# RustAudio/rodio

Measured on AMD Instinct MI355X. Metric: Msamples/s through resample+low_pass+mix pipeline, higher is better.
Workload: dtype f32; 1 GPU; 256 f32 stereo sources/GPU x 1048576 frames, 44.1->48 kHz linear resample + low_pass(200) + ordered Mixer sum, span_len=None; numpy default_rng(1234+s) U(-1,1)/256; in_frames=1048576, out_frames=1141308, channels=2, kernel=k_rlm_chunk

## Files before the change

### include/rodio_hip.h

```cpp
#ifndef RODIO_HIP_H
#define RODIO_HIP_H

#include <stddef.h>
#include <stdint.h>

#ifdef __cplusplus
extern "C" {
#endif

typedef int32_t rh_status;
enum {
    RH_OK = 0,
    RH_ERR_INVALID = 1,
    RH_ERR_HIP = 2,
    RH_ERR_UNSUPPORTED = 3,
    RH_ERR_NOMEM = 4,
    RH_ERR_TIMEOUT = 5,
    RH_ERR_NOT_INITIALIZED = 6,
    RH_ERR_CAPACITY = 7
};

typedef void *rh_stream;

int32_t rh_version(void);
// ... 172 lines not shown
    float knee_width_db;
    uint64_t attack_ns;
    uint64_t release_ns;
} rh_limit_params;
rh_status rh_limit(float *dst, const float *src, uint64_t frames, uint32_t channels,
                   uint32_t sample_rate, uint32_t n_streams, const rh_limit_params *params_host,
                   float *state, rh_stream stream);

typedef struct rh_agc_params {
    float target_level;
    uint64_t attack_ns;
    uint64_t release_ns;
    float absolute_max_gain;
    float floor;
} rh_agc_params;
size_t rh_agc_state_floats(void);
rh_status rh_agc_state_init(float *state, uint32_t n_streams, rh_stream stream);
rh_status rh_agc(float *dst, const float *src, uint64_t n_samples, uint32_t sample_rate,
                 uint32_t n_streams, const rh_agc_params *params_host, float *state,
                 rh_stream stream);

typedef struct rh_rlm_config {
    uint32_t from_rate, to_rate;
    uint32_t channels;
    uint64_t span_len;
    int32_t filter_kind;
    uint32_t filter_freq;
    float filter_q;
    uint32_t max_sources;
    uint64_t max_in_frames;
    uint32_t frames_per_lane;
    uint32_t ring_stages;
    uint32_t no_balance;
    uint32_t force_general;
    float custom_coeffs[5];
    uint32_t filter_first;
} rh_rlm_config;
typedef struct rh_rlm rh_rlm;
rh_status rh_rlm_create(rh_rlm **out, const rh_rlm_config *cfg);
rh_status rh_rlm_destroy(rh_rlm *p);
rh_status rh_rlm_set_sources(rh_rlm *p, const float *const *srcs_host,
                             const uint64_t *in_frames_host, uint32_t n_sources);
rh_status rh_rlm_set_gains(rh_rlm *p, const float *gains_host, uint32_t n);
rh_status rh_rlm_set_filters(rh_rlm *p, const int32_t *kinds_host, const uint32_t *freqs_host, const float *qs_host, uint32_t n);
rh_status rh_rlm_set_exclusive(rh_rlm *p, int32_t exclusive);
rh_status rh_rlm_set_mix_first(rh_rlm *p, int32_t enable);
rh_status rh_rlm_run(rh_rlm *p, float *dst, uint64_t out_capacity_frames, uint64_t *out_frames,
                     rh_stream stream);
rh_status rh_rlm_run_subset(rh_rlm *p, uint32_t first, uint32_t count, float *dst,
                            uint64_t out_capacity_frames, uint64_t *out_frames, rh_stream stream);
rh_status rh_rlm_stream_begin(rh_rlm *p);
rh_status rh_rlm_stream_block(rh_rlm *p, const float *const *srcs_host, uint32_t n_sources,
                              uint64_t avail_frames, int32_t flush, float *dst,
                              uint64_t out_capacity_frames, uint64_t *out_frames,
                              uint64_t *consumed_frames, rh_stream stream);
rh_status rh_rlm_stream_block_v(rh_rlm *p, const float *const *srcs_host, const uint64_t *avail_frames_host,
                                const uint8_t *ended_host, uint32_t n_sources, float *dst,
                                uint64_t out_capacity_frames, uint64_t *out_frames,
                                uint64_t *consumed_frames, rh_stream stream);
rh_status rh_rlm_stream_keep_history(rh_rlm *p, int32_t on);
rh_status rh_rlm_stream_overlap(rh_rlm *p, int32_t on);
rh_status rh_rlm_stream_one_launch_blocks(rh_rlm *p, uint32_t *blocks);
rh_status rh_rlm_stream_overlapped_blocks(rh_rlm *p, uint32_t *blocks);
rh_status rh_rlm_stream_stats(rh_rlm *p, uint32_t *summed_blocks, uint32_t *per_source_blocks, uint32_t *recoveries);
rh_status rh_rlm_run_batch(rh_rlm *p, float *dst, uint64_t dst_stride_frames, uint64_t *out_frames,
                           rh_stream stream);
rh_status rh_rlm_autotune(rh_rlm *p, float *dst, uint64_t out_capacity_frames, rh_stream stream,
                          uint32_t *frames_per_lane, uint32_t *ring_stages);
rh_status rh_rlm_last_status(rh_rlm *p);
rh_status rh_rlm_late_carries(rh_rlm *p, uint64_t *count);
rh_status rh_rlm_phase_cycles(rh_rlm *p, double out8[8]);
typedef struct rh_rlm_geometry_info {
    uint32_t threads;
    uint32_t frames_per_lane;
    uint32_t ring_stages;
    uint32_t stage_kib;
    uint32_t lds_bytes;
    uint32_t lookback_tiles;
    uint32_t resident_waves_per_cu;
    uint32_t n_tiles;
    uint32_t general_kernel;
    uint32_t ragged_pair;
    uint32_t mix_first;
} rh_rlm_geometry_info;
rh_status rh_rlm_geometry(rh_rlm *p, rh_rlm_geometry_info *info);

enum { RH_GEN_SINE = 0, RH_GEN_TRIANGLE = 1, RH_GEN_SQUARE = 2, RH_GEN_SAWTOOTH = 3 };
rh_status rh_signal_generator_init(float state_host[2], uint32_t sample_rate, float frequency);
rh_status rh_signal_generator_seek(float *phase_host, uint32_t sample_rate, float frequency, uint64_t pos_ns);
float rh_signal_phase_advance(float phase, float phase_step, uint64_t n);
rh_status rh_signal_generate(float *dst, uint64_t ld, uint64_t n, float *states_dev, const int32_t *functions_dev,
                             uint32_t n_gens, rh_stream stream);
rh_status rh_chirp_total_samples(uint32_t sample_rate, uint64_t duration_ns, uint64_t *total);
rh_status rh_chirp_total_duration(uint32_t sample_rate, uint64_t total, uint64_t *secs, uint32_t *nanos);
rh_status rh_chirp(float *dst, uint64_t first, uint64_t n, uint64_t total, uint32_t sample_rate, float start_frequency,
                   float end_frequency, uint64_t *out_n, rh_stream stream);

enum {
    RH_NOISE_WHITE_UNIFORM = 0,
    RH_NOISE_WHITE_TRIANGULAR = 1,
    RH_NOISE_WHITE_GAUSSIAN = 2,
    RH_NOISE_PINK = 3,
    RH_NOISE_BLUE = 4,
    RH_NOISE_VIOLET = 5,
    RH_NOISE_BROWNIAN = 6,
    RH_NOISE_RED = 7,
    RH_NOISE_VELVET = 8
};
rh_status rh_noise_init(uint32_t state_host[8], int32_t kind, uint32_t sample_rate, uint64_t seed, uint32_t density);
rh_status rh_noise_generate(float *dst, uint64_t ld, uint64_t n, uint32_t *states_dev, uint32_t n_streams, rh_stream stream);

typedef struct rh_comm rh_comm;
rh_status rh_comm_unique_id(uint8_t out128[128]);
rh_status rh_comm_init(rh_comm **out, int32_t rank, int32_t nranks, const uint8_t uid128[128]);
rh_status rh_comm_destroy(rh_comm *c);
rh_status rh_allreduce_sum_f32(rh_comm *c, float *buf, size_t n, rh_stream stream);
rh_status rh_reduce_sum_f32(rh_comm *c, float *buf, size_t n, int32_t root, rh_stream stream);

#ifdef __cplusplus
}
#endif
#endif
```

### rodio_amd/_lib.py

```python
from __future__ import annotations

import ctypes as C
import os

_HERE = os.path.dirname(os.path.abspath(__file__))
LIB_PATH = os.environ.get("RODIO_HIP_LIB") or os.path.join(_HERE, "librodio_hip.so")

RH_OK = 0
STATUS_NAMES = {
    0: "RH_OK", 1: "RH_ERR_INVALID", 2: "RH_ERR_HIP", 3: "RH_ERR_UNSUPPORTED", 4: "RH_ERR_NOMEM",
    5: "RH_ERR_TIMEOUT", 6: "RH_ERR_NOT_INITIALIZED", 7: "RH_ERR_CAPACITY",
}


class RhError(RuntimeError):
    def __init__(self, status: int, where: str, detail: str = ""):
        self.status = status
        super().__init__(f"{where}: {STATUS_NAMES.get(status, status)} {detail}".strip())


class LimitParams(C.Structure):
    _fields_ = [("threshold_db", C.c_float), ("knee_width_db", C.c_float),
                ("attack_ns", C.c_uint64), ("release_ns", C.c_uint64)]


class AgcParams(C.Structure):
    _fields_ = [("target_level", C.c_float), ("attack_ns", C.c_uint64), ("release_ns", C.c_uint64),
                ("absolute_max_gain", C.c_float), ("floor", C.c_float)]


class WavInfo(C.Structure):
    _fields_ = [("channels", C.c_uint32), ("sample_rate", C.c_uint32), ("bits_per_sample", C.c_uint32), ("is_float", C.c_int32),
                ("data_offset", C.c_uint64), ("data_bytes", C.c_uint64), ("samples", C.c_uint64)]


class UniformSeg(C.Structure):
    _fields_ = [("src", C.c_void_p), ("dst", C.c_void_p), ("src_frame0", C.c_uint64), ("src_frames", C.c_uint64), ("m0", C.c_uint64), ("m1", C.c_uint64),
                ("span_frames", C.c_uint64), ("from_rate", C.c_uint32), ("to_rate", C.c_uint32), ("from_ch", C.c_uint32), ("to_ch", C.c_uint32), ("gain", C.c_float), ("reserved", C.c_uint32)]


class WideSrc(C.Structure):
    _fields_ = [("data", C.c_void_p), ("channels", C.c_uint32), ("from_rate", C.c_uint32), ("phase", C.c_uint32), ("frames", C.c_uint64), ("last", C.c_uint32), ("gain", C.c_float)]


class RlmConfig(C.Structure):
    _fields_ = [("from_rate", C.c_uint32), ("to_rate", C.c_uint32), ("channels", C.c_uint32),
                ("span_len", C.c_uint64), ("filter_kind", C.c_int32), ("filter_freq", C.c_uint32),
                ("filter_q", C.c_float), ("max_sources", C.c_uint32), ("max_in_frames", C.c_uint64),
                ("frames_per_lane", C.c_uint32), ("ring_stages", C.c_uint32), ("no_balance", C.c_uint32), ("force_general", C.c_uint32), ("custom_coeffs", C.c_float * 5), ("filter_first", C.c_uint32)]


class RlmGeometry(C.Structure):
    _fields_ = [(n, C.c_uint32) for n in ("threads", "frames_per_lane", "ring_stages", "stage_kib", "lds_bytes",
                                           "lookback_tiles", "resident_waves_per_cu", "n_tiles", "general_kernel", "ragged_pair", "mix_first")]


vp, sz, u32, u64, i32, f32 = C.c_void_p, C.c_size_t, C.c_uint32, C.c_uint64, C.c_int32, C.c_float
f32p = C.POINTER(C.c_float)

SIGNATURES = {
    "rh_version": (i32, []),
    "rh_status_string": (C.c_char_p, [i32]),
    "rh_last_hip_error": (C.c_char_p, []),
    "rh_async_status": (i32, []),
    "rh_init": (i32, [i32]),
    "rh_device_name": (i32, [C.c_char_p, sz]),
    "rh_bind_thread": (i32, []),
    "rh_malloc": (i32, [C.POINTER(vp), sz]),
    "rh_free": (i32, [vp]),
    "rh_memset": (i32, [vp, i32, sz, vp]),
    "rh_memcpy_h2d": (i32, [vp, vp, sz, vp]),
    "rh_memcpy_h2d_rows": (i32, [vp, vp, sz, sz, sz, vp]),
    "rh_memcpy_d2h": (i32, [vp, vp, sz, vp]),
    "rh_memcpy_d2h_async": (i32, [vp, vp, C.c_size_t, vp]),
    "rh_memcpy_d2d": (i32, [vp, vp, C.c_size_t, vp]),
    "rh_host_alloc": (i32, [C.POINTER(vp), C.c_size_t]),
    "rh_host_free": (i32, [vp]),
    "rh_event_synchronize": (i32, [vp]),
    "rh_stream_wait_event": (i32, [vp, vp]),
    "rh_stream_create": (i32, [C.POINTER(vp)]),
    "rh_stream_destroy": (i32, [vp]),
    "rh_stream_synchronize": (i32, [vp]),
    "rh_stream_release_scratch": (i32, [vp]),
    "rh_event_create": (i32, [C.POINTER(vp)]),
    "rh_event_destroy": (i32, [vp]),
    "rh_event_record": (i32, [vp, vp]),
    "rh_event_elapsed_ms": (i32, [vp, vp, f32p]),
    "rh_convert_i8_to_f32": (i32, [vp, vp, sz, vp]),
    "rh_convert_u8_to_f32": (i32, [vp, vp, sz, vp]),
    "rh_convert_i16_to_f32": (i32, [vp, vp, sz, vp]),
    "rh_convert_u16_to_f32": (i32, [vp, vp, sz, vp]),
    "rh_convert_i24_to_f32": (i32, [vp, vp, sz, vp]),
    "rh_convert_i32_to_f32": (i32, [vp, vp, sz, vp]),
    "rh_convert_f32_to_i8": (i32, [vp, vp, sz, vp]),
    "rh_convert_f32_to_i16": (i32, [vp, vp, sz, vp]),
    "rh_convert_f32_to_u16": (i32, [vp, vp, sz, vp]),
    "rh_convert_f32_to_i32": (i32, [vp, vp, sz, vp]),
    "rh_convert_f32_to_u8": (i32, [vp, vp, sz, vp]),
    "rh_convert_f32_to_i24": (i32, [vp, vp, sz, vp]),
    "rh_convert_f32_to_u24": (i32, [vp, vp, sz, vp]),
    "rh_convert_f32_to_u32": (i32, [vp, vp, sz, vp]),
    "rh_convert_f32_to_i64": (i32, [vp, vp, sz, vp]),
    "rh_convert_f32_to_u64": (i32, [vp, vp, sz, vp]),
    "rh_convert_f32_to_f64": (i32, [vp, vp, sz, vp]),
    "rh_convert_u24_to_f32": (i32, [vp, vp, sz, vp]),
    "rh_convert_u32_to_f32": (i32, [vp, vp, sz, vp]),
    "rh_convert_i64_to_f32": (i32, [vp, vp, sz, vp]),
    "rh_convert_u64_to_f32": (i32, [vp, vp, sz, vp]),
    "rh_convert_f64_to_f32": (i32, [vp, vp, sz, vp]),
    "rh_channels_convert": (i32, [vp, vp, sz, u32, u32, vp]),
    "rh_amplify": (i32, [vp, vp, sz, f32, vp]),
    "rh_channel_volume": (i32, [vp, vp, sz, u32, f32p, u32, vp]),
    "rh_spatial_gains": (i32, [f32p, f32p, f32p, f32p]),
    "rh_periodic_update_samples": (u64, [u64, u32, u32]),
    "rh_amplify_steps": (i32, [vp, vp, sz, u64, u64, vp, u32, vp]),
    "rh_channel_volume_steps": (i32, [vp, vp, sz, u32, u32, u64, u64, vp, u32, u64, u64, vp, u32, vp]),
    "rh_delay_samples": (u64, [u64, u32, u32]),
    "rh_echo_mix": (i32, [vp, vp, sz, sz, f32, vp]),
    "rh_resample_out_frames": (i32, [u64, u32, u32, u32, u64, C.POINTER(u64)]),
    "rh_resample_linear": (i32, [vp, vp, u64, u32, u32, u32, u64, vp]),
    "rh_uniform_span_frames": (i32, [u64, u32, u32, i32, C.POINTER(u64)]),
    "rh_uniform_first_tap": (i32, [u64, u32, u32, C.POINTER(u64)]),
    "rh_uniform_cut_tail_samples": (i32, [u64, u32, u32, u32, u32, u32, C.POINTER(u64)]),
    "rh_uniform_segments": (i32, [C.POINTER(UniformSeg), u32, vp]),
    "rh_uniform_segments_dev": (i32, [vp, u32, u64, vp]),
    "rh_mix_sum": (i32, [vp, sz, C.POINTER(vp), C.POINTER(u64), C.POINTER(u64), u32, vp]),
    "rh_wide_mix_block": (i32, [vp, u32, u32, u64, C.POINTER(WideSrc), u32, vp]),
    "rh_biquad_coeffs": (i32, [i32, u32, f32, u32, f32p]),
    "rh_biquad": (i32, [vp, vp, u64, u32, u32, f32p, vp, i32, vp]),
    "rh_limit": (i32, [vp, vp, u64, u32, u32, u32, C.POINTER(LimitParams), vp, vp]),
    "rh_agc_state_floats": (sz, []),
    "rh_agc_state_init": (i32, [vp, u32, vp]),
    "rh_agc": (i32, [vp, vp, u64, u32, u32, C.POINTER(AgcParams), vp, vp]),
    "rh_resampler_create": (i32, [C.POINTER(vp), u32, u32, u32]),
    "rh_resampler_reset": (i32, [vp]),
    "rh_resampler_destroy": (i32, [vp]),
    "rh_resampler_pending_frames": (i32, [vp, u64, i32, C.POINTER(u64)]),
# ... 86 lines not shown
```

### rodio_amd/csrc/rh_common.h

```cpp
#pragma once
#include <mutex>
#include <hip/hip_runtime.h>

#include <cstdint>
#include <cstdio>

#include "../../include/rodio_hip.h"

namespace rh {

extern bool g_initialized;
extern int g_device;
extern int g_num_cus;
extern uint32_t *g_async_status;
void set_hip_error(hipError_t e, const char *what);

enum Knob {
    K_AGC_SEQ, K_AGC_VEC, K_BIQUAD_NO_FALLBACK, K_BIQUAD_SEQ, K_BIQUAD_R, K_BIQUAD_NW, K_BIQUAD_WGS, K_LIMIT_SEQ, K_LIMIT_R, K_LIMIT_NW, K_LIMIT_WGS, K_LIMIT_GRID,
    K_LIMIT_SKEW, K_LIMIT_NIO, K_LIMIT_INIT, K_SCAN_DMA_TOP, K_SCAN_SPIN_LIMIT, K_NO_HYBRID, K_NO_TICKET_SHARDS, K_PROF_DUMP, K_HOST_ALLOC, K_NO_MIX_FIRST, K_MIX_U, K_NO_CHUNK, K_CHUNK_HALF, K_AUTOTUNE_LOG, K_RAG_RESIDENT, K_RAG_TWO_KERNELS, K_AGC_SEGMENTS, K_RS_PIPE, K_DASP_I64_VIA_F64, K_MIX_GROUPS, K_CLASSES_SIDE_BY_SIDE, K_AGC_FUSED_R4, K_STREAM_UPLOAD_ALWAYS, K_STREAM_NO_REJOIN, K_NO_SBLK, K_SBLK_KV, K_SBLK_NO_OVERLAP, K_CLASSES_ONE_BY_ONE, K_CLASSES_ONE_WAVE, K_WIDE_GENERAL, K_PCM_NO_TILE, K_PCM_TILE_KB, K_LERP_IEEE_DIV, K_COUNTER_JUMP, K_STREAM_START, K_COUNT
};
const char *knob(Knob k);
void load_knobs();
struct CounterJump {
    bool on;
    uint32_t after, tickets_left, launches_left;
};
const CounterJump &counter_jump();
bool scan_jump_due();

#define RH_HIP_TRY(expr)                                   \
    do {                                                   \
        hipError_t _e = (expr);                            \
        if (_e != hipSuccess) {                            \
            ::rh::set_hip_error(_e, #expr);                \
            return RH_ERR_HIP;                             \
        }                                                  \
    } while (0)

#define RH_REQUIRE_INIT()                                  \
    do {                                                   \
        if (!::rh::g_initialized) return RH_ERR_NOT_INITIALIZED; \
    } while (0)

#define RH_CHECK_LAUNCH()                                  \
    do {                                                   \
        hipError_t _e = hipGetLastError();                 \
        if (_e != hipSuccess) {                            \
            ::rh::set_hip_error(_e, "kernel launch");      \
            return RH_ERR_HIP;                             \
        }                                                  \
    } while (0)

inline hipStream_t as_stream(rh_stream s) { return reinterpret_cast<hipStream_t>(s); }

inline hipError_t fill_now(void *p, int value, size_t bytes) {
    hipError_t e = hipMemset(p, value, bytes);
    return e != hipSuccess ? e : hipStreamSynchronize(nullptr);
}

hipError_t fill_async(void *p, int value, size_t bytes, hipStream_t s);
hipError_t counters_add(uint32_t *ctl, uint32_t d_ticket, uint32_t n_shards, uint32_t d_shards, hipStream_t s);

struct ScratchAux {
    uint64_t tag;
    uint32_t ticket_base;
    uint32_t parity;
};
hipError_t stream_scratch(hipStream_t s, size_t bytes, void **out, std::unique_lock<std::mutex> &hold, ScratchAux **aux = nullptr);
hipError_t copy_d2d(void *dst, const void *src, size_t bytes, hipStream_t hs);
bool lerp_div_fast_ok(uint32_t T);
inline float lerp_rcp(uint32_t T) { return lerp_div_fast_ok(T) ? 1.0f / (float)T : 0.0f; }
bool pcm_tile_try(float *dst, const uint8_t *data, uint64_t n_samples, uint64_t frames, uint32_t channels, uint32_t to_channels, int fmt, hipStream_t s);
void rlm_stream_retired(hipStream_t s);

inline unsigned grid_for(size_t work_items, unsigned block = 256, unsigned max_blocks = 256 * 8) {
    size_t b = (work_items + block - 1) / block;
    if (b < 1) b = 1;
    if (b > max_blocks) b = max_blocks;
    return static_cast<unsigned>(b);
}

inline unsigned grid_tiles(size_t vectors, unsigned block = 256) { return grid_for(vectors, block, 1u << 22); }

#ifdef __HIPCC__
typedef float nt_f4 __attribute__((ext_vector_type(4)));
typedef unsigned nt_u4 __attribute__((ext_vector_type(4)));
__device__ __forceinline__ float4 ld_nt(const float4 *p) {
    const nt_f4 v = __builtin_nontemporal_load(reinterpret_cast<const nt_f4 *>(p));
    return make_float4(v.x, v.y, v.z, v.w);
}
__device__ __forceinline__ uint4 ld_nt(const uint4 *p) {
    const nt_u4 v = __builtin_nontemporal_load(reinterpret_cast<const nt_u4 *>(p));
    return make_uint4(v.x, v.y, v.z, v.w);
}
__device__ __forceinline__ float ld_nt(const float *p) { return __builtin_nontemporal_load(p); }
__device__ __forceinline__ void st_nt(float4 *p, float4 v) {
    nt_f4 t;
    t.x = v.x; t.y = v.y; t.z = v.z; t.w = v.w;
    __builtin_nontemporal_store(t, reinterpret_cast<nt_f4 *>(p));
}
__device__ __forceinline__ void st_nt(float *p, float v) { __builtin_nontemporal_store(v, p); }

// ... 49 lines not shown
```

### rodio_amd/csrc/rh_pipeline.hip

```cpp
#include "rh_pipeline_dev.h"

namespace {


__device__ __forceinline__ uint32_t rag_find_pairs(const Params &p, const uint32_t m_tile0, const uint32_t m_stable, const int lane, lds_u8 *lds, const uint32_t list_off);
template <int R, int KV, int C>
__device__ __forceinline__ void rag_run_pairs(const Params &p, unsigned long long *const rows, const uint32_t tile, const uint32_t n_pairs, const int lane, lds_u8 *lds, const uint32_t lds0,
                                              const uint32_t list_off, const uint32_t i_base, const uint32_t nvec, const uint32_t (&goff)[KV], const int (&offA)[R + 2], const float (&wgt)[R + 2],
                                              const float (&lM)[4], const float (&b15)[4], const float (&b31)[4], const float (&kM)[4], typename Chan<C>::V (&acc)[R]);

template <int R, int KV, int NS, bool FILT, bool RAG = false, int C = 2, bool SUMF = false>
__global__ __launch_bounds__(64, (R <= 4 ? (KV <= 5 ? 5 : 4) : R <= 6 ? 3 : R <= 12 ? 2 : 1)) void k_rlm_fast(const Params p) {
    typedef Chan<C> CH;
    typedef typename CH::V V;
    constexpr uint32_t FB = CH::kFB, VF = CH::kVF;
    static_assert(R <= kMaxR, "frames per lane");
    static_assert(NS >= 2 && NS <= 4, "ring depth");
    static_assert(KV * (NS - 1) < 64, "vmcnt range");
    constexpr uint32_t kStage = KV * 1024;
    extern __shared__ __attribute__((aligned(16))) unsigned char smem[];
    lds_u8 *const lds = (lds_u8 *)smem;
    const uint32_t lds0 = (uint32_t)(uintptr_t)lds;

    const int lane = threadIdx.x;
// ... 1194 lines not shown
    for (int k = 0; k < KV; ++k) acc[k] = v4f{0.f, 0.f, 0.f, 0.f};
    if (v0 < nvec) {
#pragma unroll
        for (int d = 0; d < NS - 1; ++d)
            if ((uint32_t)d < n_sources) stage_source(d, d);
        uint32_t st = 0;
        float g_next = n_sources ? dgain[4] : 0.f;
        for (uint32_t s_ = 0; s_ < n_sources; ++s_) {
            const float g = g_next;
            g_next = s_ + 1 < n_sources ? dgain[8 * (uint64_t)(s_ + 1) + 4] : 0.f;
            if (s_ + NS - 1 < n_sources) {
                uint32_t into = st + NS - 1;
                into = into >= (uint32_t)NS ? into - NS : into;
                stage_source(s_ + NS - 1, into);
                wait_vm<KV *(NS - 1)>();
            } else {
                const uint32_t left = n_sources - 1 - s_;
                wait_groups<KV, NS>((int)left);
            }
            const lds_u8 *buf = lds + st * kStage;
            v4f v[KV];
#pragma unroll
            for (int k = 0; k < KV; ++k) v[k] = *(const lds_f4 *)(buf + k * 1024 + lane * 16);
            asm volatile("s_waitcnt lgkmcnt(0)" ::: "memory");
#pragma unroll
            for (int k = 0; k < KV; ++k) {
                acc[k].x = fma_(g, v[k].x, acc[k].x);
                acc[k].y = fma_(g, v[k].y, acc[k].y);
                acc[k].z = fma_(g, v[k].z, acc[k].z);
                acc[k].w = fma_(g, v[k].w, acc[k].w);
            }
            st = st + 1 == (uint32_t)NS ? 0 : st + 1;
        }
        wait_vm<0>();
#pragma unroll
        for (int k = 0; k < KV; ++k) {
            const uint64_t j = v0 + (uint64_t)k * 64 + lane;
            if (j < nvec) *reinterpret_cast<v4f *>(y + 4 * j) = acc[k];
        }
    }
    if (blockIdx.x == 0) {
        const uint64_t t = nvec * 4 + lane;
        if (t < n_floats) {
            float a = 0.f;
            for (uint32_t s_ = 0; s_ < n_sources; ++s_) a = fma_(dgain[8 * (uint64_t)s_ + 4], ((glb_cf32 *)(uintptr_t)(desc[4 * (uint64_t)s_] + src_off))[t], a);
            y[t] = a;
        }
        if (lane == 0) {
            ydesc->data = desc_row;
            ydesc->frames = frames;
            ydesc->out_frames = out_frames;
            ydesc->gain = 1.0f;
            ydesc->pad[0] = ydesc->pad[1] = ydesc->pad[2] = 0;
        }
    }
}

struct ChunkArgs {
    const uint32_t *m_lo;
    unsigned long long *halo;
    const float *lookT;
    const float *powM;
    const float *uni;
};
constexpr uint32_t kChunkMultiMax = 7;
struct ChunkMulti {
    struct Entry {
        Params p;
        ChunkArgs q;
    };
    uint32_t n;
    uint32_t first[kChunkMultiMax + 1];
    float *sum_out;
    Entry e[kChunkMultiMax];
};
static_assert(sizeof(ChunkMulti) <= 4096, "the kernarg segment");
#if defined(RH_CHUNK_DIAG) && RH_CHUNK_DIAG == 3
#define RH_CPH(i) { const unsigned long long cph_now = __builtin_readcyclecounter(); if (lane == 0) atomicAdd(p.ticket + 8 + (i), (uint32_t)(cph_now - cph_last)); cph_last = cph_now; }
#define RH_CPH_DECL unsigned long long cph_last = __builtin_readcyclecounter();
#else
#define RH_CPH(i)
#define RH_CPH_DECL
#endif
template <int R, int C, int KV>
__device__ __forceinline__ void rlm_chunk_tile(const Params &p, const ChunkArgs &q, const uint32_t block) {
    typedef Chan<C> CH;
    typedef typename CH::V V;
    constexpr int NS = 2, H = 4;
    constexpr uint32_t FB = CH::kFB;
    constexpr uint32_t kStage = KV * 1024, P = kStage / FB;
    constexpr uint32_t MB = NS * kStage + 64;
    __shared__ __attribute__((aligned(1024))) unsigned char smem[MB + kStage + 64];
    lds_u8 *const lds = (lds_u8 *)smem;
    const uint32_t lds0 = (uint32_t)(uintptr_t)lds;
    typedef __attribute__((address_space(4))) const uint64_t cu64;
    typedef __attribute__((address_space(4))) const float cf32;
    typedef __attribute__((address_space(4))) const uint32_t cu32;
    cu64 *const desc = (cu64 *)(uintptr_t)p.srcs;
    cf32 *const dgain = (cf32 *)(uintptr_t)p.srcs;
    const int lane = threadIdx.x;
    uint32_t tile = block;
    if (!p.direct) {
        const uint32_t x = block & 7u;
        const uint32_t k = __builtin_amdgcn_readfirstlane(lane == 0 ? atomicAdd(p.ticket + 32u * (1u + x), 1u) - p.shard_base : 0u);
        tile = x + 8u * k;
        if (tile >= p.n_tiles) return;
    }
#ifdef RH_CHUNK_RAGSIM
    const uint32_t Ns = p.eq_frames;
    const uint32_t S = 2u * tile < p.n_tiles ? p.n_sources : (uint32_t)(((uint64_t)p.n_sources * 2u * (p.n_tiles - tile)) / p.n_tiles);
#else
    const uint32_t Ns = p.eq_frames, S = p.n_sources;
#endif
    const uint32_t m_lo = ((cu32 *)(uintptr_t)q.m_lo)[tile], m_hi = ((cu32 *)(uintptr_t)q.m_lo)[tile + 1];
    const uint32_t m0 = m_lo + (uint32_t)lane * R;
    int nfl;
    uint32_t n_t_v;
    float pwv[4];
    {
        const uint32_t n_t = m_hi - m_lo;
        nfl = (int)n_t - lane * R < 0 ? 0 : ((int)n_t - lane * R > R ? R : (int)n_t - lane * R);
        const uint32_t nl0 = (n_t + R - 1) / R;
        const uint32_t v = nl0 ? n_t - (nl0 - 1) * R : 0;
        n_t_v = n_t;
        asm volatile("v_mov_b32 %0, %1" : "=v"(n_t_v) : "s"(n_t));
        const float *pw = q.powM + 4 * v;
#pragma unroll
        for (int k = 0; k < 4; ++k) {
            pwv[k] = pw[k];
            asm volatile("" : "+v"(pwv[k]));
        }
    }
    const bool first = (m0 == 0);

    const uint32_t nvec = Ns * C / 4;
    const uint32_t v0 = tile * (KV * 64);
    uint32_t goff[KV];
#pragma unroll
    for (int k = 0; k < KV; ++k) {
        uint32_t j = v0 + (uint32_t)k * 64 + lane;
        j = j < nvec ? j : nvec - 1;
        goff[k] = j * 16;
    }
    const bool lin = v0 + (uint32_t)(KV * 64) <= nvec;
    auto stage_source = [&](uint32_t s_, uint32_t stage) {
        const void *data = (const void *)(uintptr_t)desc[4 * (uint64_t)s_];
        if (lin) {
            glds16_run<KV>(data, goff[0], lds0 + stage * kStage);
        } else {
#pragma unroll
            for (int k = 0; k < KV; ++k) glds16(data, goff[k], lds0 + stage * kStage + k * 1024);
        }
    };
    if (S) stage_source(0, 0);
    if (S > 1) stage_source(1, 1);
    const Tables *__restrict__ tb = p.tabs;
    float lM[4], b15[4], b31[4], kM[4];
    constexpr int NHV = H * FB / 16;
    const uint32_t Jc = p.J < tile ? p.J : tile;
    int want_look = (uint32_t)lane < Jc ? 1 : 0;
    uint64_t a_halo_pub = (uint64_t)(uintptr_t)(q.halo + (uint64_t)tile * 8 + (uint32_t)(lane >= 64 - NHV ? lane - (64 - NHV) : 0) * 4);
    uint64_t a_halo_poll = (uint64_t)(uintptr_t)(q.halo + (uint64_t)(tile ? tile - 1 : 0) * 8 + (lane < H * C ? lane : 0));
    uint64_t a_gran_pub = (uint64_t)(uintptr_t)(p.gran + (uint64_t)tile * 4 + (lane < 2 * C ? lane : 0));
    uint64_t a_gran_poll = (uint64_t)(uintptr_t)(p.gran + (uint64_t)(tile ? tile - 1 - (want_look ? lane : 0) : 0) * 4);
    uint64_t a_out = (uint64_t)(uintptr_t)(p.out + ((uint64_t)m_lo + (uint32_t)lane) * C);
    uint32_t epoch_v = p.epoch;
    float U = q.uni[lane < 61 ? lane : 60];
    asm volatile("" : "+v"(want_look), "+v"(a_halo_pub), "+v"(a_halo_poll), "+v"(a_gran_pub), "+v"(a_gran_poll), "+v"(a_out), "+v"(epoch_v), "+v"(U));
    {
        const uint32_t Jc0 = Jc;
        const float *kp = q.lookT + ((uint64_t)tile * p.J + ((uint32_t)lane < Jc0 ? lane : 0)) * 4;
#pragma unroll
        for (int k = 0; k < 4; ++k) {
            lM[k] = tb->laneM[lane][k];
            b15[k] = tb->bc15M[lane][k];
            b31[k] = tb->bc31M[lane][k];
            kM[k] = kp[k];
        }
    }
    int offA[R + 2];
    float wgt[R + 2];
    {
        const int64_t fbase = (int64_t)tile * P;
        Cursor c = cursor_at(first ? 0 : m0 - 2, p);
#pragma unroll
        for (int rr = 0; rr < R + 2; ++rr) {
#if defined(RH_CHUNK_DIAG) && RH_CHUNK_DIAG == 2
            offA[rr] = (int)MB + rr * 8;
            wgt[rr] = 0.5f;
            continue;
#endif
            const bool dummy = first && rr < 2;
            uint64_t i;
            uint32_t num;
            cursor_resolve(c, p, i, num);
            if (i + 1 >= Ns) {
                i = Ns - 1;
                num = 0;
            }
            int64_t f = (int64_t)i - fbase;
            f = f < -H ? -H : (f > (int64_t)P - 1 ? (int64_t)P - 1 : f);
            offA[rr] = dummy ? (int)MB : (int)MB + (int)f * (int)FB;
            wgt[rr] = dummy ? 0.0f : (float)num / p.Tf;
            if (!dummy) cursor_next(c, p);
        }
    }
    v4f acc[KV];
#pragma unroll
    for (int k = 0; k < KV; ++k) acc[k] = v4f{0.f, 0.f, 0.f, 0.f};
    {
        uint32_t st = 0;
        float g_next = S ? dgain[4] : 0.f;
        for (uint32_t s_ = 0; s_ < S; ++s_) {
            const float g = g_next;
            g_next = s_ + 1 < S ? dgain[8 * (uint64_t)(s_ + 1) + 4] : 0.f;
            if (s_ + 1 < S) wait_vm<KV>();
            else wait_vm<0>();
            const lds_u8 *buf = lds + st * kStage;
            v4f v[KV];
#pragma unroll
            for (int k = 0; k < KV; ++k) v[k] = *(const lds_f4 *)(buf + k * 1024 + lane * 16);
            asm volatile("s_waitcnt lgkmcnt(0)" ::: "memory");
            if (s_ + 2 < S) stage_source(s_ + 2, st);
#pragma unroll
            for (int k = 0; k < KV; ++k) {
                acc[k].x = fma_(g, v[k].x, acc[k].x);
                acc[k].y = fma_(g, v[k].y, acc[k].y);
                acc[k].z = fma_(g, v[k].z, acc[k].z);
                acc[k].w = fma_(g, v[k].w, acc[k].w);
            }
            st ^= 1u;
        }
    }
    RH_CPH_DECL
#if defined(RH_CHUNK_DIAG) && RH_CHUNK_DIAG < 3
    {
        float t = 0.f;
#pragma unroll
        for (int k = 0; k < KV; ++k) t += acc[k].x + acc[k].y + acc[k].z + acc[k].w;
#pragma unroll
        for (int rr = 0; rr < R + 2; ++rr) t += wgt[rr] + (float)offA[rr];
        p.out[(uint64_t)tile * 64 + lane] = t + lM[0] + b15[0] + b31[0] + kM[0] + (float)nfl + (first ? 1.f : 0.f);
        return;
    }
#endif
    if (lane >= 64 - NHV) {
        unsigned long long *hp = (unsigned long long *)(uintptr_t)a_halo_pub;
        const float e[4] = {acc[KV - 1].x, acc[KV - 1].y, acc[KV - 1].z, acc[KV - 1].w};
#pragma unroll
        for (int w = 0; w < 4; ++w) __hip_atomic_store(hp + w, ((unsigned long long)epoch_v << 32) | __float_as_uint(e[w]), __ATOMIC_RELAXED, __HIP_MEMORY_SCOPE_AGENT);
    }
#pragma unroll
    for (int k = 0; k < KV; ++k) *(lds_f4 *)(lds + MB + (uint32_t)(k * 64 + lane) * 16) = acc[k];
    if (lane == 0) *(lds_f4 *)(lds + MB + kStage) = v4f{0.f, 0.f, 0.f, 0.f};
    bool dead = false;
    if (tile == 0) {
        if (lane < H * C) *(RH_LDS float *)(lds + MB - H * FB + lane * 4) = 0.0f;
    } else {
        const bool want = lane < H * C;
        const unsigned long long *hp = (const unsigned long long *)(uintptr_t)a_halo_poll;
        unsigned long long hv = 0;
        bool ok = false;
        uint32_t spins = 0;
        while (true) {
            if (want && !ok) {
                hv = __hip_atomic_load(hp, __ATOMIC_RELAXED, __HIP_MEMORY_SCOPE_AGENT);
                ok = (uint32_t)(hv >> 32) == epoch_v;
            }
            if (__all(ok || !want)) break;
            if (++spins > kSpinLimit) {
                if (lane == 0) atomicOr(p.status, 1u);
                dead = true;
                break;
            }
            __builtin_amdgcn_s_sleep(1);
        }
        if (want) *(RH_LDS float *)(lds + MB - H * FB + lane * 4) = dead ? __builtin_nanf("") : __uint_as_float((uint32_t)hv);
    }
    asm volatile("s_waitcnt lgkmcnt(0)" ::: "memory");
    __builtin_amdgcn_wave_barrier();
    RH_CPH(0)

    const float b0 = readlane_f(U, 0), c1 = readlane_f(U, 1), c2 = readlane_f(U, 2), na1 = -readlane_f(U, 3), na2 = -readlane_f(U, 4);
    V out[R];
    V E1 = CH::zero(), E2 = CH::zero();
    {
        V ta[R + 2], tb2[R + 2];
#pragma unroll
        for (int rr = 0; rr < R + 2; ++rr) {
            ta[rr] = CH::ld_lds(lds + offA[rr]);
            tb2[rr] = CH::ld_lds(lds + offA[rr] + FB);
        }
        auto tap = [&](int rr) -> V {
            V x;
#pragma unroll
            for (int ch = 0; ch < C; ++ch) CH::set(x, ch, fma_(CH::get(tb2[rr], ch) - CH::get(ta[rr], ch), wgt[rr], CH::get(ta[rr], ch)));
            return x;
        };
        V x2 = first ? CH::zero() : tap(0);
        V x1 = first ? CH::zero() : tap(1);
        V w1 = CH::zero(), w2 = CH::zero();
#pragma unroll
        for (int r = 0; r < R; ++r) {
            const V x = tap(r + 2);
            V w;
#pragma unroll
            for (int ch = 0; ch < C; ++ch) {
                const float wc = fma_(na1, CH::get(w1, ch), fma_(na2, CH::get(w2, ch), fma_(c2, CH::get(x2, ch), c1 * CH::get(x1, ch))));
                CH::set(w, ch, wc);
                CH::set(out[r], ch, fma_(b0, CH::get(x, ch), wc));
            }
            w2 = w1;
            w1 = w;
            x2 = x1;
            x1 = x;
            E1 = vsel(r + 1 == nfl, w1, E1);
            E2 = vsel(r + 1 == nfl, w2, E2);
        }
    }
    RH_CPH(1)
    float Pq[2 * C];
#pragma unroll
    for (int k = 0; k < 2 * C; ++k) Pq[k] = 0.f;
    {
        const float Tm[4] = {readlane_f(U, 5), readlane_f(U, 6), readlane_f(U, 7), readlane_f(U, 8)};
#pragma unroll
        for (int ch = 0; ch < C; ++ch) mat_acc(Tm, CH::get(E1, ch), CH::get(E2, ch), Pq[2 * ch], Pq[2 * ch + 1]);
    }
    float own[2 * C];
#pragma unroll
    for (int k = 0; k < 2 * C; ++k) own[k] = Pq[k];
#define RH_CSCAN(K, N)                                                                             \
    {                                                                                              \
        float sq[2 * C];                                                                           \
        _Pragma("unroll") for (int k = 0; k < 2 * C; ++k) sq[k] = dpp0<kDppRowShr + N, 0xf>(Pq[k]); \
        const float sM[4] = {readlane_f(U, 9 + 4 * K), readlane_f(U, 10 + 4 * K), readlane_f(U, 11 + 4 * K), readlane_f(U, 12 + 4 * K)}; \
        _Pragma("unroll") for (int ch = 0; ch < C; ++ch) mat_acc(sM, sq[2 * ch], sq[2 * ch + 1], Pq[2 * ch], Pq[2 * ch + 1]); \
    }
    RH_CSCAN(0, 1)
    RH_CSCAN(1, 2)
    RH_CSCAN(2, 4)
    RH_CSCAN(3, 8)
#undef RH_CSCAN
    {
        float sq[2 * C];
#pragma unroll
        for (int k = 0; k < 2 * C; ++k) sq[k] = dpp0<kDppBcast15, 0xa>(Pq[k]);
#pragma unroll
        for (int ch = 0; ch < C; ++ch) mat_acc(b15, sq[2 * ch], sq[2 * ch + 1], Pq[2 * ch], Pq[2 * ch + 1]);
    }
    {
        float sq[2 * C];
#pragma unroll
        for (int k = 0; k < 2 * C; ++k) sq[k] = dpp0<kDppBcast31, 0xc>(Pq[k]);
#pragma unroll
        for (int ch = 0; ch < C; ++ch) mat_acc(b31, sq[2 * ch], sq[2 * ch + 1], Pq[2 * ch], Pq[2 * ch + 1]);
    }
    {
        const uint32_t n_t = (uint32_t)__builtin_amdgcn_readfirstlane((int)n_t_v);
        const int nl = (int)((n_t + R - 1) / R);
        float A[2 * C];
#pragma unroll
        for (int k = 0; k < 2 * C; ++k) A[k] = 0.f;
        if (nl >= 1) {
#pragma unroll
            for (int k = 0; k < 2 * C; ++k) A[k] = __int_as_float(__builtin_amdgcn_readlane(__float_as_int(own[k]), nl - 1));
        }
        if (nl >= 2) {
            const float M[4] = {readfirstlane_f(pwv[0]), readfirstlane_f(pwv[1]), readfirstlane_f(pwv[2]), readfirstlane_f(pwv[3])};
            float xp[2 * C];
#pragma unroll
            for (int k = 0; k < 2 * C; ++k) xp[k] = __int_as_float(__builtin_amdgcn_readlane(__float_as_int(Pq[k]), nl - 2));
#pragma unroll
            for (int ch = 0; ch < C; ++ch) mat_acc(M, xp[2 * ch], xp[2 * ch + 1], A[2 * ch], A[2 * ch + 1]);
        }
        if (lane < 2 * C) {
            float ev = A[0];
#pragma unroll
            for (int k = 1; k < 2 * C; ++k) ev = lane == k ? A[k] : ev;
            __hip_atomic_store((unsigned long long *)(uintptr_t)a_gran_pub, ((unsigned long long)epoch_v << 32) | __float_as_uint(ev), __ATOMIC_RELAXED, __HIP_MEMORY_SCOPE_AGENT);
        }
    }
    float Q[2 * C];
#pragma unroll
    for (int k = 0; k < 2 * C; ++k) Q[k] = dpp0<kDppWaveShr1, 0xf>(Pq[k]);
    RH_CPH(2)
    float c[2 * C];
#pragma unroll
    for (int k = 0; k < 2 * C; ++k) c[k] = 0.f;
    if (tile > 0) {
        const bool want = want_look != 0;
        const unsigned long long *gp = (const unsigned long long *)(uintptr_t)a_gran_poll;
        unsigned long long gv[2 * C];
#pragma unroll
        for (int k = 0; k < 2 * C; ++k) gv[k] = 0;
        bool ok = false;
        uint32_t spins = 0;
        while (true) {
            if (want && !ok) {
                bool all = true;
#pragma unroll
                for (int k = 0; k < 2 * C; ++k) {
                    gv[k] = __hip_atomic_load(gp + k, __ATOMIC_RELAXED, __HIP_MEMORY_SCOPE_AGENT);
                    all = all && ((uint32_t)(gv[k] >> 32) == epoch_v);
                }
                ok = all;
            }
            if (__all(ok || !want)) break;
            if (++spins > kSpinLimit) {
                if (lane == 0) atomicOr(p.status, 1u);
                dead = true;
                break;
            }
            __builtin_amdgcn_s_sleep(4);
        }
        if (lane == 0 && spins) atomicAdd(p.status + 1, spins);
        if (want && ok && !dead) {
#pragma unroll
            for (int ch = 0; ch < C; ++ch) mat_acc(kM, __uint_as_float((uint32_t)gv[2 * ch]), __uint_as_float((uint32_t)gv[2 * ch + 1]), c[2 * ch], c[2 * ch + 1]);
        }
#pragma unroll
        for (int k = 0; k < 2 * C; ++k) {
            c[k] += dpp0<kDppRowShr + 1, 0xf>(c[k]);
            c[k] += dpp0<kDppRowShr + 2, 0xf>(c[k]);
            c[k] += dpp0<kDppRowShr + 4, 0xf>(c[k]);
            c[k] += dpp0<kDppRowShr + 8, 0xf>(c[k]);
            c[k] = readlane_f(c[k], 15) + readlane_f(c[k], 31);
        }
    }
    if (dead) {
#pragma unroll
        for (int k = 0; k < 2 * C; ++k) c[k] = __builtin_nanf("");
    }
    RH_CPH(3)
#pragma unroll
    for (int ch = 0; ch < C; ++ch) mat_acc(lM, c[2 * ch], c[2 * ch + 1], Q[2 * ch], Q[2 * ch + 1]);
    constexpr uint32_t kRow = (R + 1) * FB;
    {
        lds_u8 *row = lds + (uint32_t)lane * kRow;
#pragma unroll
        for (int r = 0; r < R; ++r) {
            V y;
#pragma unroll
            for (int ch = 0; ch < C; ++ch) CH::set(y, ch, fma_(readlane_f(U, 25 + 2 * r), Q[2 * ch], fma_(readlane_f(U, 26 + 2 * r), Q[2 * ch + 1], CH::get(out[r], ch))));
            if (C == 2) *(lds_f2 *)(row + r * FB) = v2f{CH::get(y, 0), CH::get(y, C - 1)};
            else *(RH_LDS float *)(row + r * FB) = CH::get(y, 0);
        }
    }
    asm volatile("s_waitcnt lgkmcnt(0)" ::: "memory");
    __builtin_amdgcn_wave_barrier();
    {
        const uint32_t n_t = (uint32_t)__builtin_amdgcn_readfirstlane((int)n_t_v);
        float *ot = (float *)(uintptr_t)a_out;
        for (uint32_t f0 = 0; f0 < n_t; f0 += 64) {
            const uint32_t f = f0 + (uint32_t)lane;
            if (f < n_t) {
                const lds_u8 *src2 = lds + (f / R) * kRow + (f % R) * FB;
                if (C == 2) {
                    const v2f a = *(const lds_f2 *)src2;
                    *reinterpret_cast<float2 *>(ot + (uint64_t)f0 * 2) = make_float2(a.x, a.y);
                } else {
                    ot[f0] = *(const RH_LDS float *)src2;
                }
            }
        }
    }
    RH_CPH(4)
}
template <int R, int C, int KV>
__global__ __launch_bounds__(64, 2) void k_rlm_chunk(const Params p, const ChunkArgs q) {
    rlm_chunk_tile<R, C, KV>(p, q, blockIdx.x);
}
template <int R, int C, int KV>
__global__ __launch_bounds__(64, 2) void k_rlm_chunk_multi(const ChunkMulti m) {
    uint32_t k = 0;
#pragma unroll
    for (uint32_t i = 1; i < kChunkMultiMax; ++i) k += (i < m.n && blockIdx.x >= m.first[i]) ? 1u : 0u;
    uint32_t b0 = 0;
#pragma unroll
    for (uint32_t i = 1; i < kChunkMultiMax; ++i) b0 = (i == k) ? m.first[i] : b0;
    k = __builtin_amdgcn_readfirstlane(k);
    typedef const __attribute__((address_space(4))) unsigned char *cbytes;
    cbytes e = (cbytes)__builtin_amdgcn_kernarg_segment_ptr() + offsetof(ChunkMulti, e) + (size_t)k * sizeof(ChunkMulti::Entry);
    Params p;
    ChunkArgs q;
    typedef const __attribute__((address_space(4))) uint32_t *cwords;
    static_assert(sizeof(Params) % 4 == 0 && sizeof(ChunkArgs) % 4 == 0 && offsetof(ChunkMulti::Entry, q) % 4 == 0, "copied word by word");
    {
        cwords wp = (cwords)(e + offsetof(ChunkMulti::Entry, p)), wq = (cwords)(e + offsetof(ChunkMulti::Entry, q));
        uint32_t *dp = reinterpret_cast<uint32_t *>(&p), *dq = reinterpret_cast<uint32_t *>(&q);
#pragma unroll
        for (uint32_t i = 0; i < sizeof(Params) / 4; ++i) dp[i] = wp[i];
#pragma unroll
        for (uint32_t i = 0; i < sizeof(ChunkArgs) / 4; ++i) dq[i] = wq[i];
    }
    rlm_chunk_tile<R, C, KV>(p, q, blockIdx.x - b0);
}

#if defined(RH_CLS_DIAG) && RH_CLS_DIAG == 9
__device__ unsigned long long g_cls_stamp[2048 * 8 * 8];
#define RH_CLS_STAMP(i) { if (lane == 0 && tile < 2048 && k < 8) g_cls_stamp[((uint64_t)tile * 8 + k) * 8 + (i)] = wall_clock64(); }
#else
#define RH_CLS_STAMP(i)
#endif
#define RH_PARG(T, e, f) (*(const __attribute__((address_space(4))) T *)((e) + offsetof(ChunkMulti::Entry, p) + offsetof(Params, f)))
#define RH_QARG(T, e, f) (*(const __attribute__((address_space(4))) T *)((e) + offsetof(ChunkMulti::Entry, q) + offsetof(ChunkArgs, f)))
template <int R, int C, int KV>
__global__ __launch_bounds__(128, 2) void k_rlm_chunk_classes(const ChunkMulti m) {
    typedef Chan<C> CH;
    typedef typename CH::V V;
    constexpr int NS = 2, H = 4;
    constexpr uint32_t FB = CH::kFB;
    constexpr uint32_t kStage = KV * 1024, P = kStage / FB;
    constexpr uint32_t kCtl = NS * kStage;
    constexpr uint32_t kImg = kStage + 128;
    constexpr uint32_t MB0 = kCtl + 64 + 64;
    __shared__ __attribute__((aligned(1024))) unsigned char smem[kCtl + 64 + 2 * kImg];
    lds_u8 *const lds = (lds_u8 *)smem;
    const uint32_t lds0 = (uint32_t)(uintptr_t)lds;
    typedef __attribute__((address_space(4))) const uint64_t cu64;
    typedef __attribute__((address_space(4))) const float cf32;
    typedef __attribute__((address_space(4))) const uint32_t cu32;
    typedef const __attribute__((address_space(4))) unsigned char *cbytes;
    const cbytes kseg = (cbytes)__builtin_amdgcn_kernarg_segment_ptr();
    const int wave = __builtin_amdgcn_readfirstlane((int)(threadIdx.x >> 6));
    const int lane = (int)(threadIdx.x & 63u);
    const uint32_t n_cls = m.n;
    const Params &p0 = m.e[0].p;
    const uint32_t tile = blockIdx.x;
    const uint32_t Ns = p0.eq_frames;
    auto entry = [&](uint32_t k) -> cbytes { return kseg + offsetof(ChunkMulti, e) + (size_t)k * sizeof(ChunkMulti::Entry); };
    auto ctl_read = [&](uint32_t which) -> uint32_t {
        uint32_t v;
        asm volatile("ds_read_b32 %0, %1\n\ts_waitcnt lgkmcnt(0)" : "=v"(v) : "v"(lds0 + kCtl + which * 4) : "memory");
        return (uint32_t)__builtin_amdgcn_readfirstlane((int)v);
    };
    auto ctl_write = [&](uint32_t which, uint32_t v) {
        asm volatile("s_waitcnt lgkmcnt(0)" ::: "memory");
        if (lane == 0) *(RH_LDS uint32_t *)(lds + kCtl + which * 4) = v;
        asm volatile("s_waitcnt lgkmcnt(0)" ::: "memory");
    };
    if (wave == 0) {
        if (lane < 2) *(RH_LDS uint32_t *)(lds + kCtl + lane * 4) = 0u;
    }
    asm volatile("s_waitcnt lgkmcnt(0)\n\ts_barrier" ::: "memory");
    if (wave == 0) {
        const uint32_t nvec = Ns * C / 4;
        const uint32_t v0 = tile * (KV * 64);
        uint32_t goff[KV];
#pragma unroll
        for (int k = 0; k < KV; ++k) {
            uint32_t j = v0 + (uint32_t)k * 64 + lane;
            j = j < nvec ? j : nvec - 1;
            goff[k] = j * 16;
        }
        const bool lin = v0 + (uint32_t)(KV * 64) <= nvec;
        auto stage_source = [&](cu64 *desc, uint32_t s_, uint32_t stage) {
            const void *data = (const void *)(uintptr_t)desc[4 * (uint64_t)s_];
            if (lin) {
                glds16_run<KV>(data, goff[0], lds0 + stage * kStage);
            } else {
#pragma unroll
                for (int k = 0; k < KV; ++k) glds16(data, goff[k], lds0 + stage * kStage + k * 1024);
            }
        };
        constexpr int NHV = H * FB / 16;
        __builtin_amdgcn_s_setprio(3);
        uint32_t kc = 0, sc = 0;
        cu64 *ndesc = (cu64 *)(uintptr_t)RH_PARG(uint64_t, entry(0), srcs);
        uint32_t nS = RH_PARG(uint32_t, entry(0), n_sources);
        uint32_t nstage = 0;
        auto request_next = [&]() {
            if (kc >= n_cls) return false;
            stage_source(ndesc, sc, nstage);
            nstage ^= 1u;
            if (++sc == nS) {
                sc = 0;
                if (++kc < n_cls) {
                    ndesc = (cu64 *)(uintptr_t)RH_PARG(uint64_t, entry(kc), srcs);
// ... 735 lines not shown

const void *chunk_kernel(int R, uint32_t channels, int KV) {
    if (channels == 2 && R == 9 && KV == 4) return reinterpret_cast<const void *>(&k_rlm_chunk<9, 2, 4>);
    if (channels == 2 && R == 18 && KV == 8) return reinterpret_cast<const void *>(&k_rlm_chunk<18, 2, 8>);
    if (channels == 2 && R == 18 && KV == 4) return reinterpret_cast<const void *>(&k_rlm_chunk<18, 2, 4>);
    if (channels == 1 && R == 18 && KV == 4) return reinterpret_cast<const void *>(&k_rlm_chunk<18, 1, 4>);
    if (channels == 1 && R == 18 && KV == 2) return reinterpret_cast<const void *>(&k_rlm_chunk<18, 1, 2>);
    return nullptr;
}

static const void *chunk_multi_kernel(int R, uint32_t channels, int KV) {
    if (channels == 2 && R == 9 && KV == 4) return reinterpret_cast<const void *>(&k_rlm_chunk_multi<9, 2, 4>);
    if (channels == 2 && R == 18 && KV == 8) return reinterpret_cast<const void *>(&k_rlm_chunk_multi<18, 2, 8>);
    if (channels == 2 && R == 18 && KV == 4) return reinterpret_cast<const void *>(&k_rlm_chunk_multi<18, 2, 4>);
    if (channels == 1 && R == 18 && KV == 4) return reinterpret_cast<const void *>(&k_rlm_chunk_multi<18, 1, 4>);
    if (channels == 1 && R == 18 && KV == 2) return reinterpret_cast<const void *>(&k_rlm_chunk_multi<18, 1, 2>);
    return nullptr;
}

static const void *chunk_classes_kernel(int R, uint32_t channels, int KV) {
    if (channels == 2 && R == 18 && KV == 8) return reinterpret_cast<const void *>(&k_rlm_chunk_classes<18, 2, 8>);
    if (channels == 2 && R == 18 && KV == 4) return reinterpret_cast<const void *>(&k_rlm_chunk_classes<18, 2, 4>);
    if (channels == 1 && R == 18 && KV == 4) return reinterpret_cast<const void *>(&k_rlm_chunk_classes<18, 1, 4>);
    if (channels == 1 && R == 18 && KV == 2) return reinterpret_cast<const void *>(&k_rlm_chunk_classes<18, 1, 2>);
    return nullptr;
}

rh_status chunk_launch_classes(rh_rlm *const *classes, float *const *rows, uint64_t row_capacity_frames, uint32_t n, float *dst_sum, rh_stream stream, bool *taken, bool *summed) {
    *taken = false;
    *summed = false;
    if (n < 2 || n > kChunkMultiMax || rh::knob(rh::K_CLASSES_ONE_BY_ONE)) return RH_OK;
    const void *fn = nullptr;
    for (uint32_t k = 0; k < n; ++k) {
        const rh_rlm *h = classes[k];
        if (!h || !h->cls.empty() || !h->plan || h->out_frames == 0 || row_capacity_frames < h->out_frames) return RH_OK;
        if (!h->chunk.ok || !mix_first_applies(h, *h->plan, h->n_sources, false, false)) return RH_OK;
        const void *f = chunk_multi_kernel(h->chunk.R, h->cfg.channels, h->chunk.KV);
        if (!f || (fn && f != fn)) return RH_OK;
        fn = f;
    }
    ChunkMulti m;
    memset(&m, 0, sizeof m);
    for (uint32_t k = 0; k < n; ++k) {
        rh_rlm *h = classes[k];
        h->collect = &m;
        const rh_status st = rlm_launch(h, 0, h->n_sources, rows[k], row_capacity_frames, nullptr, stream, 0, 0, StreamArgs{});
        h->collect = nullptr;
        if (st != RH_OK) return st;
        if (m.n != k + 1) return RH_ERR_UNSUPPORTED;
    }
    void *args[] = {&m};
    hipStream_t s = rh::as_stream(stream);
    const void *fn2 = rh::knob(rh::K_CLASSES_ONE_WAVE) ? nullptr : chunk_classes_kernel(classes[0]->chunk.R, classes[0]->cfg.channels, classes[0]->chunk.KV);
    bool same = fn2 != nullptr;
    for (uint32_t k = 0; k < n && same; ++k) {
        const rh_rlm *h = classes[k], *h0 = classes[0];
        same = h->exclusive && h->eq_frames == h0->eq_frames && h->out_frames == h0->out_frames && h->F == h0->F && h->T == h0->T && h->chunk_in == h0->chunk_in &&
               h->chunk_out == h0->chunk_out && h->chunk.n_tiles == h0->chunk.n_tiles && h->chunk.R == h0->chunk.R && h->chunk.KV == h0->chunk.KV && h->n_sources >= 1;
    }
    if (same) {
        int per_cu = 0;
        same = hipOccupancyMaxActiveBlocksPerMultiprocessor(&per_cu, fn2, 128, 0) == hipSuccess && per_cu >= 1 &&
               (uint64_t)classes[0]->chunk.n_tiles <= (uint64_t)per_cu * (uint64_t)rh::g_num_cus;
    }
    hipError_t e;
    if (same) {
        m.sum_out = dst_sum;
        e = hipLaunchKernel(fn2, dim3(classes[0]->chunk.n_tiles), dim3(128), args, 0, s);
        *summed = e == hipSuccess;
    } else {
        e = hipLaunchKernel(fn, dim3(m.first[m.n]), dim3(64), args, 0, s);
        if (e == hipSuccess)
            for (uint32_t k = 0; k < n; ++k) classes[k]->shard_base += (m.first[k + 1] - m.first[k]) / 8u;
    }
    if (e != hipSuccess) {
        rh::set_hip_error(e, "k_rlm_chunk_multi / k_rlm_chunk_classes launch");
        return RH_ERR_HIP;
    }
    for (uint32_t k = 0; k < n; ++k) mark_launch(classes[k], s);
    *taken = true;
    return RH_OK;
}

#if defined(RH_CLS_DIAG) && RH_CLS_DIAG == 9
extern "C" int rh_debug_cls_stamps(unsigned long long *dst, size_t n) {
    return (int)hipMemcpyFromSymbol(dst, HIP_SYMBOL(g_cls_stamp), n * sizeof(unsigned long long), 0, hipMemcpyDeviceToHost);
}
#endif
void launch_state(hipStream_t s, unsigned long long *gran, const Tables *tabs, uint32_t n_sources, uint32_t cols, uint32_t last_col, uint32_t J, uint32_t epoch, uint32_t next_epoch) {
    hipLaunchKernelGGL(k_rlm_state, dim3((n_sources + 63) / 64), dim3(64), 0, s, gran, tabs, n_sources, cols, last_col, J, epoch, next_epoch);
}

void launch_state_sum(hipStream_t s, const unsigned long long *gran, const SrcDesc *srcs, uint32_t n_sources, uint32_t cols, uint32_t tag, float *w_out) {
    hipLaunchKernelGGL(k_rlm_state_sum, dim3(1), dim3(256), 0, s, gran, srcs, n_sources, cols, tag, w_out);
}

bool mix_first_applies(const rh_rlm *p, const Plan &pl, uint32_t count, bool per_source_states, bool batch) {
    return &pl == &p->fast && p->filt && p->mix_first_on && !per_source_states && !batch && count >= 2 && !rh::knob(rh::K_NO_MIX_FIRST);
}

rh_status rlm_launch(rh_rlm *p, uint32_t first, uint32_t count, float *dst, uint64_t out_capacity_frames, uint64_t *out_frames, rh_stream stream, uint32_t batch_streams, uint64_t out_stride,
                            const StreamArgs &sa) {
    RH_REQUIRE_INIT();
    if (!p) return RH_ERR_INVALID;
    if (!p->cls.empty()) return RH_ERR_UNSUPPORTED;
    if (first > p->n_sources || count > p->n_sources - first) return RH_ERR_INVALID;
    if (out_frames) *out_frames = p->out_frames;
    if (p->out_frames == 0) return RH_OK;
    if (!dst || (reinterpret_cast<uintptr_t>(dst) & 15u)) return RH_ERR_INVALID;
    if (out_capacity_frames < p->out_frames) return RH_ERR_CAPACITY;
    hipStream_t s = rh::as_stream(stream);
    {
        const rh_status w = pre_launch(p, s);
        if (w != RH_OK) return w;
    }
    const Plan &pl = *p->plan;
    {
        const rh_status w = next_epoch(p, s);
        if (w != RH_OK) return w;
    }
    Params k;
    k.srcs = p->d_srcs + first;
    k.tabs = pl.d_tabs;
    k.out = dst;
    k.gran = p->d_gran;
    k.ticket = p->d_ctl;
    k.status = p->d_ctl + 1;
    k.out_frames = p->out_frames;
    k.chunk_in = sa.mode ? p->st_chunk_in : p->chunk_in;
    k.chunk_out = sa.mode ? p->st_chunk_out : p->chunk_out;
    k.n_sources = count;
    k.n_tiles = p->n_tiles;
    k.F = p->F;
    k.T = p->T;
    k.qF = p->F / p->T;
    k.rF = p->F % p->T;
    k.Tf = (float)p->T;
    k.rcpT = rh::lerp_rcp(p->T);
    k.epoch = p->epoch;
    k.J = pl.J;
    k.ticket_base = p->ticket_base;
    k.direct = 0;
    k.rag_merge = k.rag_pairs_from = k.rag_pairs_to = 0;
    k.prof = p->d_prof;
    k.eq_frames = p->eq_frames;
    k.batch_streams = batch_streams;
    k.shards = (batch_streams >= 16 && batch_streams % 8 == 0 && !rh::knob(rh::K_NO_TICKET_SHARDS)) ? 8u : 1u;
    k.shard_base = p->shard_base;
    k.out_stride = out_stride;
    k.st_mode = sa.mode;
    k.st_active = sa.active;
    k.st_m0 = sa.m0;
    k.st_g0 = sa.g0;
    k.st_mfirst = sa.mode ? p->st_mfirst : 0;
    k.st_win = sa.win;
    k.st_wout = sa.wout;
    k.gran_cols = sa.gran_cols ? sa.gran_cols : p->n_tiles;
    k.col0 = sa.gran_cols ? 1u : 0u;
    k.u = pl.uni;
    void *args[] = {&k};
    const uint64_t grid = (uint64_t)p->n_tiles * (batch_streams ? batch_streams : 1);
    if (grid > 0x7fffffffull) return RH_ERR_UNSUPPORTED;
    if (&pl == &p->pair && !sa.mode && !batch_streams) {
        Params k1 = k;
        k1.gran = p->d_gran + (uint64_t)count * p->n_tiles * 4;
        k1.eq_frames = p->rag_frames;
        void *args1[] = {&k1};
#ifdef RH_RAG_NO_SUMF
        const bool merge = false;
#else
        const bool merge = !rh::knob(rh::K_RAG_TWO_KERNELS) || !pl.v->plain;
#endif
        k1.rag_merge = merge ? 1u : 0u;
        k1.rag_pairs_from = p->rag_pairs_from;
        k1.rag_pairs_to = p->rag_pairs_to;
        uint32_t lds1 = pl.lds_bytes + 128u;
        if (const char *w = rh::knob(rh::K_RAG_RESIDENT)) {
            const int want = atoi(w);
            if (want >= 2 && want < 8) lds1 = std::max(lds1, (kLdsGranules / (uint32_t)want) * kLdsGranule);
        }
        const uint32_t grid8 = ((uint32_t)grid + 7u) & ~7u;
        k1.shards = 8;
        k1.shard_base = p->shard_base;
        hipError_t e1 = hipLaunchKernel(reinterpret_cast<const void *>(pl.v->filt), dim3(grid8), dim3(64), args1, lds1, s);
        if (e1 == hipSuccess) p->shard_base += grid8 / 8u;
        if (e1 == hipSuccess && !merge) {
            k.ticket_base = p->ticket_base;
            e1 = hipLaunchKernel(reinterpret_cast<const void *>(pl.v->plain), dim3((uint32_t)grid), dim3(64), args, 2u * (uint32_t)pl.v->KV * 1024u + 128u , s);
            p->ticket_base += (uint32_t)grid;
        }
        if (e1 != hipSuccess) {
            rh::set_hip_error(e1, "ragged batch launch");
            return RH_ERR_HIP;
        }
        return mark_launch(p, s);
    }
    if (p->chunk.ok && !sa.mode && mix_first_applies(p, pl, count, false, batch_streams != 0) && count == p->n_sources && first == 0) {
        const ChunkPlan &c = p->chunk;
        k.tabs = c.d_tabs;
        k.gran = c.d_gran;
        k.n_tiles = c.n_tiles;
        k.J = c.J;
        k.u = c.uni;
        ChunkArgs ca;
        ca.m_lo = c.d_mlo;
        ca.halo = c.d_halo;
        ca.lookT = c.d_look;
        ca.powM = c.d_pow;
        ca.uni = c.d_uni;
        k.direct = (c.direct && p->exclusive) ? 1u : 0u;
        if (p->collect) {
            ChunkMulti &m = *static_cast<ChunkMulti *>(p->collect);
            if (m.n >= kChunkMultiMax) return RH_ERR_UNSUPPORTED;
            k.direct = 0;
            const uint32_t g8 = (c.n_tiles + 7u) & ~7u;
            m.e[m.n].p = k;
            m.e[m.n].q = ca;
            m.first[m.n + 1] = m.first[m.n] + g8;
            m.n += 1;
            return RH_OK;
        }
        const uint32_t cgrid = k.direct ? c.n_tiles : (c.n_tiles + 7u) & ~7u;
        void *cargs[] = {&k, &ca};
        const hipError_t ce = hipLaunchKernel(c.fn, dim3(cgrid), dim3(64), cargs, 0, s);
        if (ce != hipSuccess) {
            rh::set_hip_error(ce, "k_rlm_chunk launch");
            return RH_ERR_HIP;
        }
        if (!k.direct) p->shard_base += cgrid / 8u;
        return mark_launch(p, s);
    }
    const bool pre = p->pre_filter;
    if (pre && (&pl != &p->fast || sa.mode || batch_streams)) return RH_ERR_UNSUPPORTED;
    if (pre || mix_first_applies(p, pl, count, sa.gran_cols != 0, batch_streams != 0)) {
        const uint64_t n_floats = (uint64_t)p->eq_frames * p->cfg.channels;
        const size_t row = (size_t)(((sa.mode ? (uint64_t)p->cfg.max_in_frames * p->cfg.channels : n_floats) + 3) & ~3ull);
        constexpr uint32_t kMixGroups = 16;
        const uint64_t nvec = n_floats / 4;
        int U = 4;
        while (U > 1 && (nvec + 256ull * U - 1) / (256ull * U) < 2ull * (uint64_t)rh::g_num_cus) U /= 2;
        if (const char *u = rh::knob(rh::K_MIX_U)) U = atoi(u);
        const uint32_t per = 256u * (uint32_t)(U == 1 ? 1 : U == 2 ? 2 : 4);
        const uint32_t wgs = (uint32_t)std::max<uint64_t>(1, (nvec + per - 1) / per);
        const uint64_t ring_waves = (nvec + 511) / 512;
        int ring = ring_waves >= 2ull * rh::g_num_cus ? 2 : 0;
        if (const char *u = rh::knob(rh::K_MIX_U)) ring = atoi(u) >= 10 ? atoi(u) - 10 : 0;
        uint32_t groups = 1;
        const uint64_t per_cu = rh::knob(rh::K_MIX_GROUPS) ? (uint64_t)std::max(1, atoi(rh::knob(rh::K_MIX_GROUPS))) : 2ull;
        if (!pre && !ring && !rh::knob(rh::K_MIX_U))
            while (groups < kMixGroups && (uint64_t)wgs * groups < per_cu * (uint64_t)rh::g_num_cus && count / (groups * 2) >= 8) groups *= 2;
        const size_t rows_needed = pre ? 2 : (sa.mode ? kMixGroups : groups);
        const size_t need = row * rows_needed + 64 + kMixGroups * 8;
        if (need > p->mix_floats) {
            const rh_status w = wait_idle(p);
            if (w != RH_OK) return w;
            if (p->d_mix) RH_HIP_TRY(hipFree(p->d_mix));
            p->d_mix = nullptr;
            RH_HIP_TRY(hipMalloc(reinterpret_cast<void **>(&p->d_mix), need * sizeof(float)));
            p->mix_floats = need;
        }
        SrcDesc *const ydesc = reinterpret_cast<SrcDesc *>(p->d_mix + (p->mix_floats - 32 - kMixGroups * 8));
        float *const frow = pre ? p->d_mix + row : p->d_mix;
        const uint32_t nf = p->eq_frames, mf = (uint32_t)p->out_frames;
        if (ring >= 3) hipLaunchKernelGGL(k_mix_ring<3>, dim3((uint32_t)ring_waves), dim3(64), 0, s, k.srcs, count, p->d_mix, n_floats, ydesc, nf, mf, frow, sa.src_off);
        else if (ring == 2) hipLaunchKernelGGL(k_mix_ring<2>, dim3((uint32_t)ring_waves), dim3(64), 0, s, k.srcs, count, p->d_mix, n_floats, ydesc, nf, mf, frow, sa.src_off);
        else if (U == 1) hipLaunchKernelGGL(k_mix_rows<1>, dim3(wgs, groups), dim3(256), 0, s, k.srcs, count, p->d_mix, n_floats, ydesc, nf, mf, frow, (uint64_t)row, sa.src_off);
        else if (U == 2) hipLaunchKernelGGL(k_mix_rows<2>, dim3(wgs, groups), dim3(256), 0, s, k.srcs, count, p->d_mix, n_floats, ydesc, nf, mf, frow, (uint64_t)row, sa.src_off);
        else hipLaunchKernelGGL(k_mix_rows<4>, dim3(wgs, groups), dim3(256), 0, s, k.srcs, count, p->d_mix, n_floats, ydesc, nf, mf, frow, (uint64_t)row, sa.src_off);
        RH_CHECK_LAUNCH();
        if (pre) {
            const rh_status fs = rh_biquad(frow, p->d_mix, p->eq_frames, p->cfg.channels, 1, p->pre_coeffs, nullptr, 1, stream);
            if (fs != RH_OK) return fs;
        }
        k.srcs = ydesc;
        k.n_sources = groups;
        k.direct = (p->exclusive && (uint64_t)p->n_tiles <= (uint64_t)rh::g_num_cus * (uint64_t)std::max(pl.resident_per_cu, 0)) ? 1u : 0u;
    }
    hipError_t e = hipLaunchKernel(pl.kernel, dim3((uint32_t)grid), dim3(64), args, batch_streams ? std::max((uint32_t)pl.v->KV * 1024u, 64u * ((uint32_t)pl.v->R * 8u + 8u))  : p->launch_lds, s);
    if (e != hipSuccess) {
        rh::set_hip_error(e, "k_rlm launch");
        return RH_ERR_HIP;
    }
    if (k.direct) {}
    else if (k.shards > 1) p->shard_base += (uint32_t)(grid / k.shards);
    else p->ticket_base += (uint32_t)grid;
    return mark_launch(p, s);
}

}
```

### rodio_amd/csrc/rh_pipeline_internal.h

```cpp
#pragma once
#include <algorithm>
#include <cmath>
#include <cstddef>
#include <cstdio>
#include <cstdlib>
#include <cstring>
#include <mutex>
#include <numeric>
#include <type_traits>
#include <unordered_map>
#include <vector>

#include "rh_common.h"

namespace rh {
struct ResampleGeom {
    uint32_t F, T;
    uint64_t in_frames, chunk_in, chunk_out, n_chunks, last_in, out_frames;
    int fits32;
};
rh_status make_resample_geom(uint64_t in_frames, uint32_t from_rate, uint32_t to_rate, uint32_t channels, uint64_t span_len, ResampleGeom *g);
}

namespace rhp {

#ifndef RH_CARRY_DEFER
#define RH_CARRY_DEFER 2
#endif
constexpr int kMaxR = 20;
constexpr int kGroupLag = RH_CARRY_DEFER;
constexpr int kMaxLook = 32;
constexpr uint32_t kSpinLimit = 1u << 22;

struct SrcDesc {
    const float *data;
    uint32_t frames;
    uint32_t out_frames;
    float gain;
    uint32_t pad[3];
};
static_assert(sizeof(SrcDesc) == 32, "descriptor stride");

struct Uniforms {
    float b0, c1, c2, a1, a2;
    float Tm[4];
    float scanM[4][4];
    float g[kMaxR][2];
};
struct Tables {
    float bc15M[64][4];
    float bc31M[64][4];
    float laneM[64][4];
    float lookM[64][4];
};

struct Params {
    const SrcDesc *srcs;
    const Tables *tabs;
    float *out;
    unsigned long long *gran;
    uint32_t *ticket;
    uint32_t *status;
    uint64_t out_frames;
    uint64_t chunk_in, chunk_out;
    uint32_t n_sources, n_tiles;
    uint32_t F, T, qF, rF;
    float Tf, rcpT;
    uint32_t epoch, J;
    uint32_t ticket_base;
    uint32_t direct;
    unsigned long long *prof;
    uint32_t eq_frames;
    uint32_t batch_streams;
    uint32_t shards;
    uint32_t shard_base;
    uint64_t out_stride;
    uint32_t st_mode, st_active;
    uint64_t st_m0, st_g0;
    uint64_t st_mfirst;
    uint32_t gran_cols, col0;
    const float *st_win;
    float *st_wout;
    uint32_t rag_merge, rag_pairs_from, rag_pairs_to;
    Uniforms u;
};

struct M2 {
    double a, b, c, d;
};
inline M2 mul(const M2 &x, const M2 &y) { return {x.a * y.a + x.b * y.c, x.a * y.b + x.b * y.d, x.c * y.a + x.d * y.c, x.c * y.b + x.d * y.d}; }
inline M2 mpow(M2 base, uint64_t e) {
    M2 r{1, 0, 0, 1};
    while (e) {
        if (e & 1) r = mul(r, base);
        base = mul(base, base);
        e >>= 1;
    }
    return r;
}
inline void put(float *dst, const M2 &m) {
    dst[0] = (float)m.a;
    dst[1] = (float)m.b;
    dst[2] = (float)m.c;
    dst[3] = (float)m.d;
}
inline double norm(const M2 &m) { return std::fabs(m.a) + std::fabs(m.b) + std::fabs(m.c) + std::fabs(m.d); }

inline void scan_basis(double a1, double a2, M2 &T, M2 &Tinv) {
    const double disc = a1 * a1 - 4.0 * a2;
    const double re = -0.5 * a1;
    double mu, nu;
    if (disc < 0.0 && std::sqrt(-disc) * 0.5 > 1e-3) {
        mu = re;
        nu = std::sqrt(-disc) * 0.5;
    } else {
        const double sq = disc > 0.0 ? std::sqrt(disc) * 0.5 : 0.0;
        const double l1 = re + sq, l2 = re - sq;
        mu = std::fabs(l1) < std::fabs(l2) ? l1 : l2;
        nu = 1.0;
    }
    T = {1.0, -mu, 0.0, nu};
    Tinv = {1.0, mu / nu, 0.0, 1.0 / nu};
}

using KernelFn = void (*)(const Params);
struct Variant {
    int R, KV, NS;
    KernelFn filt, plain;
};
struct VariantTab {
    const Variant *v;
    size_t n;
};
template <size_t N>
constexpr VariantTab tab_of(const Variant (&t)[N]) { return VariantTab{t, N}; }
inline const Variant *find_variant(VariantTab tab, int R, int kv_needed, int NS) {
    const Variant *best = nullptr;
    for (size_t i = 0; i < tab.n; ++i) {
        const Variant &v = tab.v[i];
        if (v.R == R && v.NS == NS && v.KV >= kv_needed && (!best || v.KV < best->KV)) best = &v;
    }
    return best;
}
constexpr uint32_t kLdsGranule = 1280, kLdsGranules = 128;
inline int blocks_per_cu(const void *fn, size_t lds) {
    if (hipFuncSetAttribute(fn, hipFuncAttributeMaxDynamicSharedMemorySize, 160 * 1024 - 512) != hipSuccess) return 0;
    int n = 0;
    if (hipOccupancyMaxActiveBlocksPerMultiprocessor(&n, fn, 64, lds) != hipSuccess) return 0;
    const int by_lds = lds ? (int)(kLdsGranules / ((lds + kLdsGranule - 1) / kLdsGranule)) : n;
    return n < by_lds ? n : by_lds;
}
inline int kv_needed(uint64_t L, uint32_t F, uint32_t T, uint32_t channels) {
    const uint64_t fb = 4ull * channels, vf = 16 / fb;
    const uint64_t span = ((L + 1) * F) / T + 5 + (128 / fb - 2);
    const uint64_t nvec = span / vf + 2;
    return (int)((nvec + 63) / 64);
}

struct ChunkPlan {
    int R = 18, KV = 8;
    const void *fn = nullptr;
    int tabs_R = 0;
    bool ok = false;
    Uniforms uni;
    Tables *d_tabs = nullptr;
    float *d_pow = nullptr;
    float *d_uni = nullptr;
    uint32_t *d_mlo = nullptr;
    float *d_look = nullptr;
    unsigned long long *d_halo = nullptr;
    unsigned long long *d_gran = nullptr;
    size_t cap_tiles = 0, cap_look = 0;
    uint32_t n_tiles = 0, J = 0, frames = 0;
    int resident_per_cu = 0;
    bool direct = true;
};
struct Plan {
    const Variant *v = nullptr;
    const void *kernel = nullptr;
    bool general = false;
    uint32_t J = 0, lds_bytes = 0;
    int resident_per_cu = 0;
    Uniforms uni;
    Tables *d_tabs = nullptr;
};

struct StreamArgs {
    uint32_t mode = 0, active = 0;
    uint64_t m0 = 0, g0 = 0;
    const float *win = nullptr;
    float *wout = nullptr;
    uint32_t gran_cols = 0;
    uint64_t src_off = 0;
};
}
using namespace rhp;

struct rh_rlm {
    rh_rlm_config cfg;
    uint32_t F, T;
    uint64_t chunk_in, chunk_out;
    bool filt;
    float coeffs[5];
    Plan fast, wave;
    Plan pair;
    Plan *plan = nullptr;
    uint32_t launch_lds = 0;
    uint32_t rag_frames = 0;
    uint32_t rag_pairs_from = 0, rag_pairs_to = 0;
    uint32_t eq_frames = 0;
    bool equal = true;
    std::vector<Plan> tried;
    SrcDesc *d_srcs = nullptr;
    uint64_t srcs_version = 0;
    std::vector<const float *> st_tab_ptrs;
    uint64_t st_tab_version = ~0ull;
    unsigned long long *d_gran = nullptr;
    size_t gran_words = 0;
    uint32_t *d_ctl = nullptr;
    float *d_mix = nullptr;
    size_t mix_floats = 0;
    ChunkPlan chunk;
    bool cls_one_launch = false;
    void *collect = nullptr;
    void *sblk = nullptr;
    bool pre_filter = false;
    float pre_coeffs[5] = {1.f, 0.f, 0.f, 0.f, 0.f};
    unsigned long long *d_prof = nullptr;
    uint32_t n_sources = 0, n_tiles = 0;
    uint64_t out_frames = 0;
    uint32_t epoch = 0;
    uint32_t n_epochs = 0;
    uint32_t ticket_base = 0;
    uint32_t shard_base = 0;
    bool st_on = false, st_done = false;
    uint64_t st_g0 = 0, st_m = 0;
    uint64_t st_mfirst = 0;
    uint64_t st_chunk_in = 0, st_chunk_out = 0;
    uint32_t st_nsrc = 0;
    float *d_w[2] = {nullptr, nullptr};
    int st_cur = 0;
    std::vector<SrcDesc> h_desc;
    static constexpr int kDescRing = 4;
    SrcDesc *h_ring[kDescRing] = {nullptr, nullptr, nullptr, nullptr};
    hipEvent_t h_ring_ev[kDescRing] = {nullptr, nullptr, nullptr, nullptr};
    int h_ring_next = 0;
    std::vector<float> gains;
    std::vector<uint64_t> st_total;
    uint32_t st_cols = 0;
    bool st_history = false;
    bool st_together = false;
    bool st_dirty = false;
    bool st_decided = false;
    std::vector<const float *> st_prev_ptrs;
// ... 67 lines not shown
```

### rodio_amd/csrc/rh_pipeline_plan.hip

```cpp
#include "rh_pipeline_internal.h"

namespace {

std::mutex g_handles_mu;
std::vector<rh_rlm *> g_handles;
}

namespace rhp {

rh_status wait_idle(rh_rlm *p) {
    if (p->launched) {
        hipError_t e = hipSuccess;
        if (!p->idle_ev) e = hipEventCreateWithFlags(&p->idle_ev, hipEventDisableTiming);
        if (e == hipSuccess) e = hipEventRecord(p->idle_ev, p->last_stream);
        if (e == hipSuccess) e = hipEventSynchronize(p->idle_ev);
        if (e != hipSuccess) {
            (void)hipGetLastError();
            e = hipDeviceSynchronize();
        }
        p->launched = false;
        p->last_stream = nullptr;
        if (e != hipSuccess) {
            rh::set_hip_error(e, "wait_idle");
            return RH_ERR_HIP;
        }
    }
    return RH_OK;
}
rh_status pre_launch(rh_rlm *p, hipStream_t s) {
    if (p->launched && p->last_stream != s) return wait_idle(p);
    return RH_OK;
}
rh_status mark_launch(rh_rlm *p, hipStream_t s) {
    p->launched = true;
    p->last_stream = s;
    return RH_OK;
}

}
namespace {
__global__ void k_retag(unsigned long long *w, size_t n, uint32_t lo, uint32_t hi, uint32_t sub, uint32_t zero_below) {
    for (size_t i = (size_t)blockIdx.x * blockDim.x + threadIdx.x; i < n; i += (size_t)gridDim.x * blockDim.x) {
        const unsigned long long v = w[i];
        const uint32_t t = (uint32_t)(v >> 32);
        if (t == 0 || t > hi || (t < lo && !zero_below)) continue;
        const uint32_t u = t >= lo ? t - sub : 0u;
        w[i] = u ? ((unsigned long long)u << 32) | (v & 0xffffffffull) : 0ull;
    }
}
}
namespace rhp {
hipError_t launch_retag(unsigned long long *w, size_t n, const Retag &r, hipStream_t s) {
    if (!w || !n) return hipSuccess;
    hipLaunchKernelGGL(k_retag, dim3(rh::grid_for(n)), dim3(256), 0, s, w, n, r.lo, r.hi, r.sub, r.zero_below ? 1u : 0u);
    return hipGetLastError();
}
static rh_status retag_tables(rh_rlm *p, hipStream_t s, const Retag &r) {
    RH_HIP_TRY(launch_retag(p->d_gran, p->gran_words, r, s));
    RH_HIP_TRY(launch_retag(p->chunk.d_halo, p->chunk.cap_tiles * 8, r, s));
    RH_HIP_TRY(launch_retag(p->chunk.d_gran, p->chunk.cap_tiles * 4, r, s));
    sblk_retag(p, s, r);
    RH_CHECK_LAUNCH();
    return RH_OK;
}
rh_status next_epoch(rh_rlm *p, hipStream_t s, bool *launched) {
    if (launched) *launched = false;
    const rh::CounterJump &j = rh::counter_jump();
    if (j.on && ++p->n_epochs == j.after) {
        const uint32_t to = 0u - j.tickets_left;
        const uint32_t dt = to - p->ticket_base, ds = to - p->shard_base;
        RH_HIP_TRY(rh::counters_add(p->d_ctl, dt, 8u, ds, s));
        p->ticket_base += dt;
        p->shard_base += ds;
        const uint32_t target = kEpochLimit - (j.launches_left < kEpochLimit - 1 ? j.launches_left : kEpochLimit - 1);
        if (target > p->epoch) {
            const rh_status st = retag_tables(p, s, Retag{p->epoch + 1u, p->epoch + 1u, p->epoch - target, false});
            if (st != RH_OK) return st;
            p->epoch = target;
        }
        if (launched) *launched = true;
    }
    if (p->epoch >= kEpochLimit) {
        const rh_status st = retag_tables(p, s, Retag{kEpochShift + 1u, 0xffffffffu, kEpochShift, true});
        if (st != RH_OK) return st;
        p->epoch -= kEpochShift;
        if (launched) *launched = true;
    }
    p->epoch += 1;
    return RH_OK;
}

uint32_t look_tiles(const M2 &B, uint64_t L) {
    const M2 BL = mpow(B, L);
    M2 cur = BL;
    for (uint32_t j = 1; j <= (uint32_t)kMaxLook; ++j) {
        if (norm(cur) < 0x1p-40) return j;
        cur = mul(cur, BL);
    }
    return 0;
}
size_t lds_bytes_of(const Variant &v, bool general, uint32_t J) {
    size_t n = (size_t)v.NS * v.KV * 1024;
    if (general) n += 128 + 32 + kMaxLook * 16 + (size_t)((J + 3) / 4) * 1024;
    return n;
}

rh_status make_plan(rh_rlm *p, Plan &pl, VariantTab tab, bool general, const rh::ResampleGeom &g, uint32_t want_R, uint32_t want_NS) {
    const M2 A{-(double)p->coeffs[3], -(double)p->coeffs[4], 1.0, 0.0};
    M2 Tm, Ti;
    scan_basis((double)p->coeffs[3], (double)p->coeffs[4], Tm, Ti);
    const M2 B = mul(mul(Tm, A), Ti);
    const uint64_t M = g.out_frames ? g.out_frames : 1;
    const int cus = rh::g_num_cus;
    const double per_frame = 19.0, per_source = general ? 170.0 : 50.0;
    double best = 1e300;
    const Variant *bestV = nullptr;
    uint32_t bestJ = 0;
    for (int R = 1; R <= kMaxR; ++R) {
        if (want_R && (int)want_R != R) continue;
        const uint64_t L = 64ull * R;
        const uint32_t Jr = p->filt ? look_tiles(B, L) : 1;
        if (Jr == 0) continue;
        const uint64_t tiles = (M + L - 1) / L;
        const uint64_t per_cu = (tiles + cus - 1) / cus;
        for (int NS = 2; NS <= 4; ++NS) {
            if (want_NS && (int)want_NS != NS) continue;
            const Variant *v = find_variant(tab, R, kv_needed(L, g.F, g.T, p->cfg.channels), NS);
            if (!v) continue;
            const void *fn = reinterpret_cast<const void *>(p->filt ? v->filt : v->plain);
            const int resident = blocks_per_cu(fn, lds_bytes_of(*v, general, Jr));
            if (resident < 1) continue;
            const double passes = std::ceil((double)per_cu / resident);
            const uint64_t on_cu = std::min<uint64_t>(per_cu, resident);
            const double w = std::ceil(on_cu / 4.0);
            const double issue = 2.6 + 1.7 / std::pow(w, 1.5);
            double cost = passes * w * (per_frame * R + per_source) * issue;
            cost *= 1.0 + 0.01 * NS;
            if (general && R < 8) cost *= 1.3;
            if (cost < best) {
                best = cost;
                bestV = v;
                bestJ = Jr;
            }
// ... 107 lines not shown
        }
        if (fits) {
            R = in.R, KV = in.KV, fn = in.fn;
            break;
        }
    }
    if (!fn) return RH_OK;
    if (c.fn != fn) {
        int n = 0;
        if (hipOccupancyMaxActiveBlocksPerMultiprocessor(&n, fn, 64, 0) != hipSuccess) return RH_OK;
        c.resident_per_cu = n < 1 ? -1 : n;
        c.fn = fn;
        c.R = R;
        c.KV = KV;
    }
    if (c.resident_per_cu < 1) return RH_OK;
    c.direct = tiles <= (uint64_t)rh::g_num_cus * (uint64_t)c.resident_per_cu;
    const M2 A{-(double)p->coeffs[3], -(double)p->coeffs[4], 1.0, 0.0};
    M2 Tm, Ti;
    scan_basis((double)p->coeffs[3], (double)p->coeffs[4], Tm, Ti);
    const M2 B = mul(mul(Tm, A), Ti);
    const uint32_t J = look_tiles(B, n_min);
    if (J == 0 || J > 32) return RH_OK;
    if ((uint64_t)tiles * J * 16 > (64ull << 20)) return RH_OK;
    {
        const rh_status w = wait_idle(p);
        if (w != RH_OK) return w;
    }
    if (c.tabs_R != R) {
        if (c.d_tabs) RH_HIP_TRY(hipFree(c.d_tabs));
        if (c.d_pow) RH_HIP_TRY(hipFree(c.d_pow));
        if (c.d_uni) RH_HIP_TRY(hipFree(c.d_uni));
        c.d_tabs = nullptr, c.d_pow = nullptr, c.d_uni = nullptr, c.tabs_R = 0;
        Tables *h = new Tables();
        std::memset(h, 0, sizeof(Tables));
        Uniforms &U = c.uni;
        std::memset(&U, 0, sizeof(U));
        U.b0 = p->coeffs[0];
        U.c1 = (float)((double)p->coeffs[1] - (double)p->coeffs[0] * (double)p->coeffs[3]);
        U.c2 = (float)((double)p->coeffs[2] - (double)p->coeffs[0] * (double)p->coeffs[4]);
        U.a1 = p->coeffs[3];
        U.a2 = p->coeffs[4];
        put(U.Tm, Tm);
        for (int k = 0; k < 4; ++k) put(U.scanM[k], mpow(B, (uint64_t)R << k));
        for (int r = 0; r < R; ++r) {
            const M2 m = mul(mpow(A, r + 1), Ti);
            U.g[r][0] = (float)m.a;
            U.g[r][1] = (float)m.b;
        }
        for (int l = 0; l < 64; ++l) {
            put(h->laneM[l], mpow(B, (uint64_t)R * l));
            put(h->bc15M[l], mpow(B, (uint64_t)R * ((l & 15) + 1)));
            put(h->bc31M[l], mpow(B, (uint64_t)R * ((l & 31) + 1)));
        }
        float pw[kMaxR + 1][4];
        std::memset(pw, 0, sizeof(pw));
        for (int v = 0; v <= R; ++v) put(pw[v], mpow(B, (uint64_t)v));
        hipError_t e = hipMalloc(reinterpret_cast<void **>(&c.d_tabs), sizeof(Tables));
        if (e == hipSuccess) e = hipMemcpy(c.d_tabs, h, sizeof(Tables), hipMemcpyHostToDevice);
        if (e == hipSuccess) e = hipMalloc(reinterpret_cast<void **>(&c.d_pow), sizeof(pw));
        if (e == hipSuccess) e = hipMemcpy(c.d_pow, pw, sizeof(pw), hipMemcpyHostToDevice);
        static_assert(offsetof(Uniforms, Tm) == 20 && offsetof(Uniforms, scanM) == 36 && offsetof(Uniforms, g) == 100, "the kernel reads the Uniforms by float index");
        if (e == hipSuccess) e = hipMalloc(reinterpret_cast<void **>(&c.d_uni), sizeof(Uniforms));
        if (e == hipSuccess) e = hipMemcpy(c.d_uni, &U, sizeof(Uniforms), hipMemcpyHostToDevice);
        delete h;
        if (e != hipSuccess) {
            rh::set_hip_error(e, "k_rlm_chunk tables");
            return e == hipErrorOutOfMemory ? RH_ERR_NOMEM : RH_ERR_HIP;
        }
        c.tabs_R = R;
    }
    if ((size_t)tiles > c.cap_tiles) {
        if (c.d_mlo) RH_HIP_TRY(hipFree(c.d_mlo));
        if (c.d_halo) RH_HIP_TRY(hipFree(c.d_halo));
        if (c.d_gran) RH_HIP_TRY(hipFree(c.d_gran));
        c.d_mlo = nullptr, c.d_halo = nullptr, c.d_gran = nullptr, c.cap_tiles = 0;
        RH_HIP_TRY(hipMalloc(reinterpret_cast<void **>(&c.d_mlo), ((size_t)tiles + 1) * 4));
        RH_HIP_TRY(hipMalloc(reinterpret_cast<void **>(&c.d_halo), (size_t)tiles * 64));
        RH_HIP_TRY(hipMalloc(reinterpret_cast<void **>(&c.d_gran), (size_t)tiles * 32));
        RH_HIP_TRY(rh::fill_now(c.d_halo, 0, (size_t)tiles * 64));
        RH_HIP_TRY(rh::fill_now(c.d_gran, 0, (size_t)tiles * 32));
        c.cap_tiles = (size_t)tiles;
    }
    const size_t look_floats = (size_t)tiles * J * 4;
    if (look_floats > c.cap_look) {
        if (c.d_look) RH_HIP_TRY(hipFree(c.d_look));
        c.d_look = nullptr, c.cap_look = 0;
        RH_HIP_TRY(hipMalloc(reinterpret_cast<void **>(&c.d_look), look_floats * 4));
        c.cap_look = look_floats;
    }
    std::vector<float> look(look_floats, 0.0f);
    {
        std::unordered_map<uint64_t, M2> memo;
        for (uint64_t t = 1; t < tiles; ++t)
            for (uint32_t j = 0; j < J && j < t; ++j) {
                const uint64_t d = (uint64_t)mlo[(size_t)t] - mlo[(size_t)(t - j)];
                auto it = memo.find(d);
                if (it == memo.end()) it = memo.emplace(d, mpow(B, d)).first;
                put(&look[((size_t)t * J + j) * 4], it->second);
            }
    }
    RH_HIP_TRY(hipMemcpy(c.d_mlo, mlo.data(), mlo.size() * 4, hipMemcpyHostToDevice));
    RH_HIP_TRY(hipMemcpy(c.d_look, look.data(), look_floats * 4, hipMemcpyHostToDevice));
    c.n_tiles = (uint32_t)tiles;
    c.J = J;
    c.frames = (uint32_t)Ns;
    c.ok = true;
    return RH_OK;
}

bool pair_ok(rh_rlm *p, const Plan &pl) {
    if (!pl.v || !p->filt || p->equal || p->cfg.force_general || p->h_desc.size() != p->n_sources || rh::knob(rh::K_NO_HYBRID)) return false;
    const uint64_t M = p->out_frames, L = 64ull * pl.v->R, J = pl.J;
    const uint64_t tiles = (M + L - 1) / L;
    if (!tiles) return false;
    uint32_t frames_of_longest = 0, most = 0, ends_from = 0xffffffffu, ends_to = 0;
    std::vector<uint32_t> pairs((size_t)tiles, 0u);
    for (const SrcDesc &d : p->h_desc) {
        if (d.out_frames == M) {
            if (frames_of_longest && frames_of_longest != d.frames) return false;
            frames_of_longest = d.frames;
        } else if (d.out_frames > 0) {
            ends_from = std::min(ends_from, d.out_frames);
            ends_to = std::max(ends_to, d.out_frames);
            const uint64_t t_end = (d.out_frames - 1) / L;
            const uint64_t t_lo = (uint64_t)d.out_frames / L > J ? (uint64_t)d.out_frames / L - J : 0;
            for (uint64_t t = t_lo; t <= t_end && t < tiles; ++t) most = std::max(most, ++pairs[(size_t)t]);
        }
    }
    if (!frames_of_longest || most > 24) return false;
    p->rag_frames = frames_of_longest;
    p->rag_pairs_from = ends_from;
    p->rag_pairs_to = ends_to;
    return true;
}

rh_status activate_plan(rh_rlm *p, Plan *pl) {
    const uint64_t M = p->out_frames;
    const uint64_t L = 64ull * pl->v->R;
    const uint64_t tiles = (M + L - 1) / L;
    if (tiles > 0x7fffffffull) return RH_ERR_UNSUPPORTED;
    const size_t words = (size_t)(p->n_sources + 1) * (tiles + 1) * 4;
    if (p->filt && words > p->gran_words) {
        {
            const rh_status w = wait_idle(p);
            if (w != RH_OK) return w;
        }
        if (p->d_gran) RH_HIP_TRY(hipFree(p->d_gran));
        p->d_gran = nullptr;
        RH_HIP_TRY(hipMalloc(reinterpret_cast<void **>(&p->d_gran), words * 8));
        RH_HIP_TRY(rh::fill_now(p->d_gran, 0, words * 8));
        p->gran_words = words;
    }
#ifdef RH_PHASE_PROFILE
    if (p->d_prof) RH_HIP_TRY(hipFree(p->d_prof));
    p->d_prof = nullptr;
    RH_HIP_TRY(hipMalloc(reinterpret_cast<void **>(&p->d_prof), (tiles + 1) * 64));
    RH_HIP_TRY(rh::fill_now(p->d_prof, 0, (tiles + 1) * 64));
#endif
    p->launch_lds = pl->lds_bytes;
    if (tiles > 0 && !p->cfg.no_balance) {
        const uint64_t per_cu = (tiles + rh::g_num_cus - 1) / rh::g_num_cus;
        if ((int)per_cu <= pl->resident_per_cu) {
            uint32_t want = (uint32_t)(kLdsGranules / per_cu) * kLdsGranule;
            if (want > 64u * 1024u) want = 64u * 1024u;
            while (want > pl->lds_bytes && blocks_per_cu(pl->kernel, want) < (int)per_cu) want -= kLdsGranule;
// ... 110 lines not shown
    }
    hipError_t e = hipSuccess;
    if (st == RH_OK) {
        e = hipMalloc(reinterpret_cast<void **>(&p->d_srcs), sizeof(SrcDesc) * cfg->max_sources);
        if (e == hipSuccess) e = hipMalloc(reinterpret_cast<void **>(&p->d_ctl), 128 * 9);
        if (e == hipSuccess) e = rh::fill_now(p->d_ctl, 0, 128 * 9);
        if (e != hipSuccess) {
            rh::set_hip_error(e, "rh_rlm_create");
            st = e == hipErrorOutOfMemory ? RH_ERR_NOMEM : RH_ERR_HIP;
        }
    }
    if (st != RH_OK) {
        rh_rlm_destroy(p);
        return st;
    }
    p->plan = &p->fast;
    {
        std::lock_guard<std::mutex> lk(g_handles_mu);
        g_handles.push_back(p);
    }
    *out = p;
    return RH_OK;
}

rh_status rh_rlm_set_exclusive(rh_rlm *p, int32_t exclusive) {
    if (!p) return RH_ERR_INVALID;
    p->exclusive = exclusive != 0;
    return RH_OK;
}

rh_status rh_rlm_set_mix_first(rh_rlm *p, int32_t enable) {
    if (!p) return RH_ERR_INVALID;
    p->mix_first_on = enable != 0;
    return RH_OK;
}

rh_status rh_rlm_destroy(rh_rlm *p) {
    if (!p) return RH_OK;
    (void)wait_idle(p);
    {
        std::lock_guard<std::mutex> lk(g_handles_mu);
        g_handles.erase(std::remove(g_handles.begin(), g_handles.end(), p), g_handles.end());
    }
#if defined(RH_CHUNK_DIAG) && RH_CHUNK_DIAG == 3
    if (p->d_ctl && p->chunk.ok) {
        uint32_t h[8] = {0};
        (void)hipMemcpy(h, p->d_ctl + 8, sizeof(h), hipMemcpyDeviceToHost);
        fprintf(stderr, "chunk phases (cycles summed over tiles and launches): image+halo %u  run %u  scan+publish %u  look-back %u  correction+stores %u\n", h[0], h[1], h[2], h[3], h[4]);
    }
#endif
    for (rh_rlm::FilterClass &c : p->cls)
        if (c.h) (void)rh_rlm_destroy(c.h);
    p->cls.clear();
    for (hipStream_t st : p->cls_streams) {
        (void)hipStreamSynchronize(st);
        (void)hipStreamDestroy(st);
    }
    for (hipEvent_t e : p->cls_done) (void)hipEventDestroy(e);
    if (p->cls_fork) (void)hipEventDestroy(p->cls_fork);
    if (p->d_cls_rows) (void)hipFree(p->d_cls_rows);
    sblk_free(p);
    if (p->idle_ev) (void)hipEventDestroy(p->idle_ev);
    bool fast_in_tried = false, wave_in_tried = false, pair_in_tried = false;
    for (Plan &c : p->tried) {
        fast_in_tried = fast_in_tried || c.d_tabs == p->fast.d_tabs;
        wave_in_tried = wave_in_tried || c.d_tabs == p->wave.d_tabs;
        pair_in_tried = pair_in_tried || c.d_tabs == p->pair.d_tabs;
        if (c.d_tabs) (void)hipFree(c.d_tabs);
    }
    if (p->fast.d_tabs && !fast_in_tried) (void)hipFree(p->fast.d_tabs);
    if (p->wave.d_tabs && !wave_in_tried) (void)hipFree(p->wave.d_tabs);
    if (p->pair.d_tabs && !pair_in_tried) (void)hipFree(p->pair.d_tabs);
    if (p->d_srcs) (void)hipFree(p->d_srcs);
    if (p->d_gran) (void)hipFree(p->d_gran);
    if (p->d_ctl) (void)hipFree(p->d_ctl);
    if (p->d_mix) (void)hipFree(p->d_mix);
    if (p->chunk.d_tabs) (void)hipFree(p->chunk.d_tabs);
    if (p->chunk.d_pow) (void)hipFree(p->chunk.d_pow);
    if (p->chunk.d_uni) (void)hipFree(p->chunk.d_uni);
    if (p->chunk.d_mlo) (void)hipFree(p->chunk.d_mlo);
    if (p->chunk.d_look) (void)hipFree(p->chunk.d_look);
    if (p->chunk.d_halo) (void)hipFree(p->chunk.d_halo);
    if (p->chunk.d_gran) (void)hipFree(p->chunk.d_gran);
    if (p->d_prof) (void)hipFree(p->d_prof);
    if (p->d_replay) (void)hipFree(p->d_replay);
    for (int k = 0; k < 2; ++k)
        if (p->d_w[k]) (void)hipFree(p->d_w[k]);
    for (int k = 0; k < rh_rlm::kDescRing; ++k) {
        if (p->h_ring_ev[k]) (void)hipEventDestroy(p->h_ring_ev[k]);
        if (p->h_ring[k]) (void)hipHostFree(p->h_ring[k]);
    }
    delete p;
    return RH_OK;
}

static rh_status set_sources_impl(rh_rlm *p, const float *const *srcs_host, const uint64_t *in_frames_host, uint32_t n_sources, const hipStream_t *on_stream) {
    RH_REQUIRE_INIT();
    if (!p || (n_sources && (!srcs_host || !in_frames_host))) return RH_ERR_INVALID;
    if (n_sources > p->cfg.max_sources) return RH_ERR_CAPACITY;
    std::vector<SrcDesc> &h = p->h_desc;
    h.resize(n_sources);
    uint64_t M = 0;
    bool equal = true;
    for (uint32_t s = 0; s < n_sources; ++s) {
        if (in_frames_host[s] > p->cfg.max_in_frames) return RH_ERR_CAPACITY;
        if (in_frames_host[s] && (!srcs_host[s] || (reinterpret_cast<uintptr_t>(srcs_host[s]) & 15u))) return RH_ERR_INVALID;
        rh::ResampleGeom g;
        rh_status st = rh::make_resample_geom(in_frames_host[s], p->cfg.from_rate, p->cfg.to_rate, p->cfg.channels, p->cfg.span_len, &g);
        if (st != RH_OK) return st;
        if (g.out_frames >= (1ull << 31)) return RH_ERR_UNSUPPORTED;
        h[s] = SrcDesc{srcs_host[s], (uint32_t)in_frames_host[s], (uint32_t)g.out_frames, s < p->gains.size() ? p->gains[s] : 1.0f, {0, 0, 0}};
        if (g.out_frames > M) M = g.out_frames;
        equal = equal && in_frames_host[s] == in_frames_host[0];
    }
    if (on_stream && p->launched && p->last_stream == *on_stream) {
        if (n_sources) {
            const rh_status up = upload_descriptors(p, n_sources, *on_stream);
            if (up != RH_OK) return up;
        }
    } else {
        const rh_status w = wait_idle(p);
        if (w != RH_OK) return w;
        if (n_sources) RH_HIP_TRY(hipMemcpy(p->d_srcs, h.data(), sizeof(SrcDesc) * n_sources, hipMemcpyHostToDevice));
        p->srcs_version += 1;
    }
    p->equal = equal;
    p->eq_frames = n_sources ? (uint32_t)in_frames_host[0] : 0;
    p->n_sources = n_sources;
    p->out_frames = M;
    p->chunk.ok = false;
    if (equal && !p->cfg.force_general) {
        const rh_status st = activate_plan(p, &p->fast);
        if (st != RH_OK || on_stream) return st;
        return build_chunk(p);
    }
    return activate_plan(p, pair_ok(p, p->pair) ? &p->pair : &p->wave);
}

static rh_status set_sources_classes(rh_rlm *p, const float *const *srcs_host, const uint64_t *in_frames_host, uint32_t n_sources) {
    if (n_sources > p->cfg.max_sources) return RH_ERR_CAPACITY;
    if (n_sources && (!srcs_host || !in_frames_host)) return RH_ERR_INVALID;
    for (rh_rlm::FilterClass &c : p->cls) c.members.clear();
    p->n_sources = 0;
    p->out_frames = 0;
    const rh_rlm::FilterSpec own{p->cfg.filter_kind == 2 ? 0 : p->cfg.filter_kind, p->cfg.filter_freq, p->cfg.filter_q};
    for (uint32_t s = 0; s < n_sources; ++s) {
        const rh_rlm::FilterSpec f = s < p->filters.size() ? p->filters[s] : own;
        size_t k = 0;
        while (k < p->cls.size() && !(p->cls[k].spec == f)) ++k;
        if (k == p->cls.size()) {
            rh_rlm::FilterClass c;
            c.spec = f;
            rh_rlm_config cfg = p->cfg;
            cfg.filter_kind = f.kind < 0 ? -1 : f.kind;
            cfg.filter_freq = f.freq;
            cfg.filter_q = f.q;
            const rh_status st = rh_rlm_create(&c.h, &cfg);
            if (st != RH_OK) return st;
            p->cls.push_back(c);
        }
        p->cls[k].members.push_back(s);
    }
    uint64_t M = 0;
    std::vector<const float *> ptrs;
    std::vector<uint64_t> frames;
    std::vector<float> gains;
// ... 264 lines not shown
        st = activate_plan(p, &slot);
        if (st != RH_OK) return st;
    }
    if (frames_per_lane) *frames_per_lane = (uint32_t)p->plan->v->R;
    if (ring_stages) *ring_stages = (uint32_t)p->plan->v->NS;
    return RH_OK;
}

rh_status rh_rlm_last_status(rh_rlm *p) {
    RH_REQUIRE_INIT();
    if (!p) return RH_ERR_INVALID;
    for (rh_rlm::FilterClass &c : p->cls) {
        const rh_status st = rh_rlm_last_status(c.h);
        if (st != RH_OK) return st;
    }
    {
        const rh_status w = wait_idle(p);
        if (w != RH_OK) return w;
    }
    uint32_t ctl[2] = {0, 0};
    RH_HIP_TRY(hipMemcpy(ctl, p->d_ctl, 8, hipMemcpyDeviceToHost));
    if (ctl[1]) {
        RH_HIP_TRY(rh::fill_now(p->d_ctl + 1, 0, 4));
        return RH_ERR_TIMEOUT;
    }
    return RH_OK;
}

rh_status rh_rlm_late_carries(rh_rlm *p, uint64_t *count) {
    RH_REQUIRE_INIT();
    if (!p || !count) return RH_ERR_INVALID;
    {
        const rh_status w = wait_idle(p);
        if (w != RH_OK) return w;
    }
    uint32_t v[2] = {0, 0};
    RH_HIP_TRY(hipMemcpy(v, p->d_ctl + 2, 8, hipMemcpyDeviceToHost));
    RH_HIP_TRY(rh::fill_now(p->d_ctl + 2, 0, 8));
    *count = v[0] | ((uint64_t)v[1] << 32);
    return RH_OK;
}

rh_status rh_rlm_phase_cycles(rh_rlm *p, double out8[8]) {
    RH_REQUIRE_INIT();
    if (!p || !out8) return RH_ERR_INVALID;
    if (!p->d_prof) return RH_ERR_UNSUPPORTED;
    std::vector<unsigned long long> h((size_t)p->n_tiles * 8);
    RH_HIP_TRY(hipMemcpy(h.data(), p->d_prof, h.size() * 8, hipMemcpyDeviceToHost));
    if (const char *path = rh::knob(rh::K_PROF_DUMP)) {
        if (FILE *f = fopen(path, "wb")) {
            fwrite(h.data(), 8, h.size(), f);
            fclose(f);
        }
    }
    for (int i = 0; i < 8; ++i) out8[i] = 0.0;
    for (uint32_t t = 0; t < p->n_tiles; ++t)
        for (int i = 0; i < 8; ++i) out8[i] += (double)h[(size_t)t * 8 + i];
    for (int i = 0; i < 8; ++i) out8[i] /= p->n_tiles ? p->n_tiles : 1;
    return RH_OK;
}

rh_status rh_rlm_geometry(rh_rlm *p, rh_rlm_geometry_info *info) {
    if (!p || !info) return RH_ERR_INVALID;
    if (!p->cls.empty()) {
        const rh_rlm::FilterClass *best = nullptr;
        for (const rh_rlm::FilterClass &c : p->cls)
            if (!best || c.members.size() > best->members.size()) best = &c;
        const rh_status st = rh_rlm_geometry(best->h, info);
        if (st == RH_OK && p->cls_one_launch) info->mix_first = 3u;
        return st;
    }
    const Plan &pl = *p->plan;
    info->threads = 64;
    info->frames_per_lane = (uint32_t)pl.v->R;
    info->ring_stages = (uint32_t)pl.v->NS;
    info->stage_kib = (uint32_t)pl.v->KV;
    info->lds_bytes = p->launch_lds ? p->launch_lds : pl.lds_bytes;
    info->lookback_tiles = pl.J;
    info->resident_waves_per_cu = (uint32_t)pl.resident_per_cu;
    info->n_tiles = p->n_tiles;
    info->general_kernel = (pl.general || p->plan == &p->pair) ? 1u : 0u;
    info->ragged_pair = p->plan == &p->pair ? 1u : 0u;
    info->mix_first = (p->pre_filter && p->plan == &p->fast) ? 1u : mix_first_applies(p, pl, p->n_sources, false, false) ? (p->chunk.ok ? 2u : 1u) : 0u;
    return RH_OK;
}

}
```

### rodio_amd/csrc/rh_runtime.hip

```cpp
#include <algorithm>
#include <atomic>
#include <cstdlib>
#include <cstring>
#include <mutex>
#include <string>
#include <unordered_map>

#include "rh_common.h"

namespace rh {
bool g_initialized = false;
int g_device = -1;
int g_num_cus = 256;
uint32_t *g_async_status = nullptr;
static thread_local std::string g_last_error;
void set_hip_error(hipError_t e, const char *what) {
    g_last_error = std::string(what) + ": " + hipGetErrorString(e);
}

namespace {
const char *const kKnobNames[K_COUNT] = {"RH_AGC_SEQ", "RH_AGC_VEC", "RH_BIQUAD_NO_FALLBACK", "RH_BIQUAD_SEQ", "RH_BIQUAD_R", "RH_BIQUAD_NW", "RH_BIQUAD_WGS", "RH_LIMIT_SEQ",
                                         "RH_LIMIT_R", "RH_LIMIT_NW", "RH_LIMIT_WGS", "RH_LIMIT_GRID", "RH_LIMIT_SKEW", "RH_LIMIT_NIO", "RH_LIMIT_INIT", "RH_SCAN_DMA_TOP", "RH_SCAN_SPIN_LIMIT", "RH_NO_HYBRID",
                                         "RH_NO_TICKET_SHARDS", "RH_PROF_DUMP", "RH_HOST_ALLOC", "RH_NO_MIX_FIRST", "RH_MIX_U", "RH_NO_CHUNK", "RH_CHUNK_HALF", "RH_AUTOTUNE_LOG", "RH_RAG_RESIDENT", "RH_RAG_TWO_KERNELS", "RH_AGC_SEGMENTS", "RH_RS_PIPE", "RH_DASP_I64_VIA_F64", "RH_MIX_GROUPS", "RH_CLASSES_SIDE_BY_SIDE", "RH_AGC_FUSED_R4", "RH_STREAM_UPLOAD_ALWAYS", "RH_STREAM_NO_REJOIN", "RH_NO_SBLK", "RH_SBLK_KV", "RH_SBLK_NO_OVERLAP", "RH_CLASSES_ONE_BY_ONE", "RH_CLASSES_ONE_WAVE", "RH_WIDE_GENERAL", "RH_PCM_NO_TILE", "RH_PCM_TILE_KB", "RH_LERP_IEEE_DIV", "RH_COUNTER_JUMP", "RH_STREAM_START"};
std::string g_knob_val[K_COUNT];
bool g_knob_set[K_COUNT];
CounterJump g_jump{false, 0, 0, 0};
std::atomic<uint32_t> g_scan_launches{0};
}
void load_knobs() {
    for (int k = 0; k < K_COUNT; ++k) {
        const char *v = getenv(kKnobNames[k]);
        g_knob_set[k] = v != nullptr;
        g_knob_val[k] = v ? v : "";
    }
    g_jump = CounterJump{false, 0, 0, 0};
    g_scan_launches = 0;
    unsigned a = 0, t = 0, l = 0;
    if (g_knob_set[K_COUNTER_JUMP] && sscanf(g_knob_val[K_COUNTER_JUMP].c_str(), "%u:%u:%u", &a, &t, &l) == 3 && a >= 1) g_jump = CounterJump{true, a, t, l};
}
const char *knob(Knob k) { return g_knob_set[k] ? g_knob_val[k].c_str() : nullptr; }
const CounterJump &counter_jump() { return g_jump; }
bool scan_jump_due() { return g_jump.on && g_scan_launches.fetch_add(1) + 1 == g_jump.after; }
namespace {
__global__ void k_fill(unsigned char *p, uint32_t word, size_t n) {
    const size_t i0 = (size_t)blockIdx.x * blockDim.x + threadIdx.x, step = (size_t)gridDim.x * blockDim.x;
    const size_t head = ((4u - (reinterpret_cast<uintptr_t>(p) & 3u)) & 3u) < n ? ((4u - (reinterpret_cast<uintptr_t>(p) & 3u)) & 3u) : n;
    const size_t words = (n - head) / 4, tail0 = head + words * 4;
    uint32_t *w = reinterpret_cast<uint32_t *>(p + head);
    for (size_t i = i0; i < words; i += step) w[i] = word;
    if (i0 < head) p[i0] = (unsigned char)word;
    if (i0 < n - tail0) p[tail0 + i0] = (unsigned char)word;
}
__global__ void k_counters_add(uint32_t *ctl, uint32_t d_ticket, uint32_t n_shards, uint32_t d_shards) {
    const uint32_t i = threadIdx.x;
    if (i == 0) atomicAdd(ctl, d_ticket);
    else if (i <= n_shards) atomicAdd(ctl + 32u * i, d_shards);
}
}
namespace {
__global__ void k_lerp_div_check(float Tf, float rcpT, uint32_t *bad) {
    const uint32_t m = blockIdx.x * blockDim.x + threadIdx.x;
    const uint32_t exps[3] = {32u, 127u, 231u};
    uint32_t miss = 0;
    for (int k = 0; k < 3; ++k)
        for (uint32_t sgn = 0; sgn < 2; ++sgn) {
            const float t = __uint_as_float((sgn << 31) | (exps[k] << 23) | m);
            const float q0 = t * rcpT;
            const float rem = __builtin_fmaf(-q0, Tf, t);
            const float q = __builtin_fmaf(rem, rcpT, q0);
            miss |= __float_as_uint(q) != __float_as_uint(t / Tf);
        }
    if (miss) atomicOr(bad, 1u);
}
std::mutex g_div_mu;
std::unordered_map<uint32_t, bool> g_div_ok;
uint32_t *g_div_flag = nullptr;
}
bool lerp_div_fast_ok(uint32_t T) {
    if (T == 0 || knob(K_LERP_IEEE_DIV) || !g_initialized) return false;
    std::lock_guard<std::mutex> hold(g_div_mu);
    auto it = g_div_ok.find(T);
    if (it != g_div_ok.end()) return it->second;
    bool ok = false;
    do {
        if (!g_div_flag && hipMalloc(reinterpret_cast<void **>(&g_div_flag), 4) != hipSuccess) break;
        if (fill_now(g_div_flag, 0, 4) != hipSuccess) break;
        const float Tf = (float)T;
        hipLaunchKernelGGL(k_lerp_div_check, dim3((1u << 23) / 256), dim3(256), 0, nullptr, Tf, 1.0f / Tf, g_div_flag);
        uint32_t bad = 1;
        if (hipMemcpy(&bad, g_div_flag, 4, hipMemcpyDeviceToHost) != hipSuccess) break;
        ok = bad == 0;
    } while (false);
    g_div_ok[T] = ok;
    return ok;
}
namespace {
struct Scratch {
    void *p = nullptr;
    size_t cap = 0;
    ScratchAux aux{0, 0, 0};
};
std::mutex g_scratch_mu;
std::unordered_map<hipStream_t, Scratch> g_scratch;
}
hipError_t stream_scratch(hipStream_t s, size_t bytes, void **out, std::unique_lock<std::mutex> &hold, ScratchAux **aux) {
    hold = std::unique_lock<std::mutex>(g_scratch_mu);
// ... 275 lines not shown
```

### rust/rodio-hip/src/ffi.rs

```rust
#![allow(non_camel_case_types, dead_code)]

pub type RhStatus = i32;
pub type RhStream = *mut core::ffi::c_void;
pub const RH_OK: RhStatus = 0;
pub const RH_ERR_INVALID: RhStatus = 1;
pub const RH_ERR_HIP: RhStatus = 2;
pub const RH_ERR_UNSUPPORTED: RhStatus = 3;
pub const RH_ERR_NOMEM: RhStatus = 4;
pub const RH_ERR_TIMEOUT: RhStatus = 5;
pub const RH_ERR_NOT_INITIALIZED: RhStatus = 6;
pub const RH_ERR_CAPACITY: RhStatus = 7;
pub const RH_GEN_SINE: RhStatus = 0;
pub const RH_GEN_TRIANGLE: RhStatus = 1;
pub const RH_GEN_SQUARE: RhStatus = 2;
pub const RH_GEN_SAWTOOTH: RhStatus = 3;
pub const RH_NOISE_WHITE_UNIFORM: RhStatus = 0;
pub const RH_NOISE_WHITE_TRIANGULAR: RhStatus = 1;
pub const RH_NOISE_WHITE_GAUSSIAN: RhStatus = 2;
pub const RH_NOISE_PINK: RhStatus = 3;
pub const RH_NOISE_BLUE: RhStatus = 4;
pub const RH_NOISE_VIOLET: RhStatus = 5;
pub const RH_NOISE_BROWNIAN: RhStatus = 6;
pub const RH_NOISE_RED: RhStatus = 7;
pub const RH_NOISE_VELVET: RhStatus = 8;

#[repr(C)] pub struct RhRlm { _private: [u8; 0] }
#[repr(C)] pub struct RhEcho { _private: [u8; 0] }
#[repr(C)] pub struct RhResampler { _private: [u8; 0] }
#[repr(C)] pub struct RhComm { _private: [u8; 0] }
#[repr(C)] #[derive(Clone, Copy)] pub struct RhWavInfo {
    pub channels: u32,
    pub sample_rate: u32,
    pub bits_per_sample: u32,
    pub is_float: i32,
    pub data_offset: u64,
    pub data_bytes: u64,
    pub samples: u64,
}
#[repr(C)] #[derive(Clone, Copy)] pub struct RhUniformSeg {
    pub src: *const f32,
    pub dst: *mut f32,
    pub src_frame0: u64,
    pub src_frames: u64,
    pub m0: u64,
    pub m1: u64,
    pub span_frames: u64,
    pub from_rate: u32,
    pub to_rate: u32,
    pub from_ch: u32,
    pub to_ch: u32,
    pub gain: f32,
    pub reserved: u32,
}
#[repr(C)] #[derive(Clone, Copy)] pub struct RhWideSrc {
    pub data: *const f32,
    pub channels: u32,
    pub from_rate: u32,
    pub phase: u32,
    pub frames: u64,
    pub last: u32,
    pub gain: f32,
}
#[repr(C)] #[derive(Clone, Copy)] pub struct RhLimitParams {
    pub threshold_db: f32,
    pub knee_width_db: f32,
    pub attack_ns: u64,
    pub release_ns: u64,
}
#[repr(C)] #[derive(Clone, Copy)] pub struct RhAgcParams {
    pub target_level: f32,
    pub attack_ns: u64,
    pub release_ns: u64,
    pub absolute_max_gain: f32,
    pub floor: f32,
}
#[repr(C)] #[derive(Clone, Copy)] pub struct RhRlmConfig {
    pub from_rate: u32,
    pub to_rate: u32,
    pub channels: u32,
    pub span_len: u64,
    pub filter_kind: i32,
    pub filter_freq: u32,
    pub filter_q: f32,
    pub max_sources: u32,
    pub max_in_frames: u64,
    pub frames_per_lane: u32,
    pub ring_stages: u32,
    pub no_balance: u32,
    pub force_general: u32,
    pub custom_coeffs: [f32; 5],
    pub filter_first: u32,
}
#[repr(C)] #[derive(Clone, Copy)] pub struct RhRlmGeometryInfo {
    pub threads: u32,
    pub frames_per_lane: u32,
    pub ring_stages: u32,
    pub stage_kib: u32,
    pub lds_bytes: u32,
    pub lookback_tiles: u32,
    pub resident_waves_per_cu: u32,
    pub n_tiles: u32,
    pub general_kernel: u32,
    pub ragged_pair: u32,
    pub mix_first: u32,
}

extern "C" {
    pub fn rh_version() -> i32;
    pub fn rh_status_string(s: RhStatus) -> *const core::ffi::c_char;
    pub fn rh_last_hip_error() -> *const core::ffi::c_char;
    pub fn rh_init(device: i32) -> RhStatus;
    pub fn rh_device_name(buf: *mut core::ffi::c_char, cap: usize) -> RhStatus;
    pub fn rh_bind_thread() -> RhStatus;
    pub fn rh_async_status() -> RhStatus;
    pub fn rh_malloc(out: *mut *mut core::ffi::c_void, bytes: usize) -> RhStatus;
    pub fn rh_free(p: *mut core::ffi::c_void) -> RhStatus;
    pub fn rh_memset(p: *mut core::ffi::c_void, value: i32, bytes: usize, stream: RhStream) -> RhStatus;
    pub fn rh_memcpy_h2d(dst: *mut core::ffi::c_void, src_host: *const core::ffi::c_void, bytes: usize, stream: RhStream) -> RhStatus;
    pub fn rh_memcpy_h2d_rows(dst: *mut core::ffi::c_void, src_host: *const core::ffi::c_void, pitch_bytes: usize, width_bytes: usize, rows: usize, stream: RhStream) -> RhStatus;
    pub fn rh_memcpy_d2h(dst_host: *mut core::ffi::c_void, src: *const core::ffi::c_void, bytes: usize, stream: RhStream) -> RhStatus;
    pub fn rh_memcpy_d2h_async(dst_host: *mut core::ffi::c_void, src: *const core::ffi::c_void, bytes: usize, stream: RhStream) -> RhStatus;
    pub fn rh_memcpy_d2d(dst: *mut core::ffi::c_void, src: *const core::ffi::c_void, bytes: usize, stream: RhStream) -> RhStatus;
    pub fn rh_host_alloc(out: *mut *mut core::ffi::c_void, bytes: usize) -> RhStatus;
    pub fn rh_host_free(p: *mut core::ffi::c_void) -> RhStatus;
    pub fn rh_stream_create(out: *mut RhStream) -> RhStatus;
    pub fn rh_stream_destroy(s: RhStream) -> RhStatus;
    pub fn rh_stream_synchronize(s: RhStream) -> RhStatus;
    pub fn rh_stream_release_scratch(s: RhStream) -> RhStatus;
    pub fn rh_event_create(out: *mut *mut core::ffi::c_void) -> RhStatus;
    pub fn rh_event_destroy(ev: *mut core::ffi::c_void) -> RhStatus;
    pub fn rh_event_record(ev: *mut core::ffi::c_void, stream: RhStream) -> RhStatus;
    pub fn rh_event_synchronize(ev: *mut core::ffi::c_void) -> RhStatus;
    pub fn rh_stream_wait_event(stream: RhStream, ev: *mut core::ffi::c_void) -> RhStatus;
    pub fn rh_event_elapsed_ms(start: *mut core::ffi::c_void, stop: *mut core::ffi::c_void, ms: *mut f32) -> RhStatus;
    pub fn rh_convert_i8_to_f32(dst: *mut f32, src: *const i8, n: usize, stream: RhStream) -> RhStatus;
    pub fn rh_convert_u8_to_f32(dst: *mut f32, src: *const u8, n: usize, stream: RhStream) -> RhStatus;
    pub fn rh_convert_i16_to_f32(dst: *mut f32, src: *const i16, n: usize, stream: RhStream) -> RhStatus;
    pub fn rh_convert_u16_to_f32(dst: *mut f32, src: *const u16, n: usize, stream: RhStream) -> RhStatus;
    pub fn rh_convert_i24_to_f32(dst: *mut f32, src: *const i32, n: usize, stream: RhStream) -> RhStatus;
    pub fn rh_convert_i32_to_f32(dst: *mut f32, src: *const i32, n: usize, stream: RhStream) -> RhStatus;
    pub fn rh_convert_f32_to_i8(dst: *mut i8, src: *const f32, n: usize, stream: RhStream) -> RhStatus;
    pub fn rh_convert_f32_to_i16(dst: *mut i16, src: *const f32, n: usize, stream: RhStream) -> RhStatus;
    pub fn rh_convert_f32_to_u16(dst: *mut u16, src: *const f32, n: usize, stream: RhStream) -> RhStatus;
    pub fn rh_convert_f32_to_i32(dst: *mut i32, src: *const f32, n: usize, stream: RhStream) -> RhStatus;
    pub fn rh_convert_f32_to_u8(dst: *mut u8, src: *const f32, n: usize, stream: RhStream) -> RhStatus;
    pub fn rh_convert_f32_to_i24(dst: *mut i32, src: *const f32, n: usize, stream: RhStream) -> RhStatus;
    pub fn rh_convert_f32_to_u24(dst: *mut i32, src: *const f32, n: usize, stream: RhStream) -> RhStatus;
    pub fn rh_convert_f32_to_u32(dst: *mut u32, src: *const f32, n: usize, stream: RhStream) -> RhStatus;
    pub fn rh_convert_f32_to_i64(dst: *mut i64, src: *const f32, n: usize, stream: RhStream) -> RhStatus;
    pub fn rh_convert_f32_to_u64(dst: *mut u64, src: *const f32, n: usize, stream: RhStream) -> RhStatus;
    pub fn rh_convert_f32_to_f64(dst: *mut f64, src: *const f32, n: usize, stream: RhStream) -> RhStatus;
    pub fn rh_convert_u24_to_f32(dst: *mut f32, src: *const i32, n: usize, stream: RhStream) -> RhStatus;
    pub fn rh_convert_u32_to_f32(dst: *mut f32, src: *const u32, n: usize, stream: RhStream) -> RhStatus;
    pub fn rh_convert_i64_to_f32(dst: *mut f32, src: *const i64, n: usize, stream: RhStream) -> RhStatus;
    pub fn rh_convert_u64_to_f32(dst: *mut f32, src: *const u64, n: usize, stream: RhStream) -> RhStatus;
    pub fn rh_convert_f64_to_f32(dst: *mut f32, src: *const f64, n: usize, stream: RhStream) -> RhStatus;
    pub fn rh_wav_probe_host(bytes: *const u8, size: usize, info: *mut RhWavInfo) -> RhStatus;
    pub fn rh_wav_decode(dst: *mut f32, data: *const u8, n_samples: u64, channels: u32, bits_per_sample: u32, is_float: i32, out_samples: *mut u64, stream: RhStream) -> RhStatus;
    pub fn rh_wav_decode_channels(dst: *mut f32, data: *const u8, n_samples: u64, channels: u32, bits_per_sample: u32, is_float: i32, to_channels: u32, out_samples: *mut u64, stream: RhStream) -> RhStatus;
    pub fn rh_wav_header_f32_host(out: *mut u8, cap: usize, channels: u32, sample_rate: u32, n_samples: u64) -> usize;
    pub fn rh_channels_convert(dst: *mut f32, src: *const f32, frames: usize, from_ch: u32, to_ch: u32, stream: RhStream) -> RhStatus;
    pub fn rh_amplify(dst: *mut f32, src: *const f32, n: usize, factor: f32, stream: RhStream) -> RhStatus;
    pub fn rh_distortion(dst: *mut f32, src: *const f32, n: usize, gain: f32, threshold: f32, stream: RhStream) -> RhStatus;
    pub fn rh_dither(dst: *mut f32, src: *const f32, n: usize, sample_offset: u64, channels: u32, target_bits: u32, algorithm: i32, seed: u64, stream: RhStream) -> RhStatus;
    pub fn rh_linear_gain_ramp(dst: *mut f32, src: *const f32, n: usize, sample_offset: u64, channels: u32, sample_rate: u32, duration_ns: u64, start_gain: f32, end_gain: f32, clamp_end: i32, stream: RhStream) -> RhStatus;
    pub fn rh_delay(dst: *mut f32, src: *const f32, n: u64, delay_samples: u64, stream: RhStream) -> RhStatus;
    pub fn rh_take_duration(dst: *mut f32, src: *const f32, n: u64, sample_offset: u64, channels: u32, sample_rate: u32, duration_ns: u64, fade_out: i32, out_samples: *mut u64, ended: *mut i32, stream: RhStream) -> RhStatus;
    pub fn rh_take_duration_from(dst: *mut f32, src: *const f32, n: u64, remaining_ns: u64, requested_ns: u64, frame_phase: u32, channels: u32, sample_rate: u32, fade_out: i32, out_samples: *mut u64, ended: *mut i32, remaining_after_ns: *mut u64, stream: RhStream) -> RhStatus;
    pub fn rh_channel_volume(dst: *mut f32, src: *const f32, frames: usize, in_ch: u32, gains_host: *const f32, out_ch: u32, stream: RhStream) -> RhStatus;
    pub fn rh_spatial_gains(emitter: *const f32, left_ear: *const f32, right_ear: *const f32, out_gains: *mut f32) -> RhStatus;
    pub fn rh_periodic_update_samples(period_ns: u64, sample_rate: u32, channels: u32) -> u64;
    pub fn rh_amplify_steps(dst: *mut f32, src: *const f32, n: usize, first: u64, period: u64, factors_dev: *const f32, n_factors: u32, stream: RhStream) -> RhStatus;
    pub fn rh_channel_volume_steps(dst: *mut f32, src: *const f32, frames: usize, in_ch: u32, out_ch: u32, first: u64, gain_period: u64, gains_dev: *const f32, n_gains: u32, factor_first: u64, factor_period: u64, factors_dev: *const f32, n_factors: u32, stream: RhStream) -> RhStatus;
    pub fn rh_delay_samples(delay_ns: u64, sample_rate: u32, channels: u32) -> u64;
    pub fn rh_echo_mix(dst: *mut f32, src: *const f32, n: usize, delay_samples: usize, gain: f32, stream: RhStream) -> RhStatus;
    pub fn rh_reverb_spatial(dst: *mut f32, src: *const f32, n: usize, delay_samples: usize, gain: f32, gains_dev: *const f32, n_streams: u32, src_stride: usize, dst_stride: usize, stream: RhStream) -> RhStatus;
    pub fn rh_resample_out_frames(in_frames: u64, from_rate: u32, to_rate: u32, channels: u32, span_len: u64, out_frames: *mut u64) -> RhStatus;
    pub fn rh_resample_linear(dst: *mut f32, src: *const f32, in_frames: u64, from_rate: u32, to_rate: u32, channels: u32, span_len: u64, stream: RhStream) -> RhStatus;
    pub fn rh_uniform_span_frames(span_in_frames: u64, from_rate: u32, to_rate: u32, complete: i32, out_frames: *mut u64) -> RhStatus;
    pub fn rh_uniform_first_tap(out_frame: u64, from_rate: u32, to_rate: u32, in_frame: *mut u64) -> RhStatus;
    pub fn rh_uniform_cut_tail_samples(span_whole_frames: u64, tail_samples: u32, from_rate: u32, to_rate: u32, from_ch: u32, to_ch: u32, out_samples: *mut u64) -> RhStatus;
    pub fn rh_uniform_segments(segs_host: *const RhUniformSeg, n_segs: u32, stream: RhStream) -> RhStatus;
    pub fn rh_uniform_segments_dev(segs_dev: *const RhUniformSeg, n_segs: u32, max_out_frames: u64, stream: RhStream) -> RhStatus;
    pub fn rh_resampler_create(out: *mut *mut RhResampler, from_rate: u32, to_rate: u32, channels: u32) -> RhStatus;
    pub fn rh_resampler_reset(p: *mut RhResampler) -> RhStatus;
    pub fn rh_resampler_destroy(p: *mut RhResampler) -> RhStatus;
    pub fn rh_resampler_pending_frames(p: *mut RhResampler, in_frames: u64, flush: i32, out_frames: *mut u64) -> RhStatus;
// ... 57 lines not shown
```

Baseline: 1.680 million Msamples/s.

## Add work-stealing takeover of half a chunk tile's source rows in k_rlm_chunk

Adds a mailbox-based work-stealing scheme to the chunked resample/low-pass/mix kernel. Tiles that finish their own work pick a still-running victim tile from a bitmap and request a takeover. The victim, if enough sources remain, hands over half of its sub-row accumulators through global slots. The thief sums the remaining sources for that half and writes the partial sums back. The goal is to cut tail imbalance when there are few tiles per CU. In exchange it adds atomic polling, extra global traffic, register pressure from the TAKE template path, and new buffer allocations.

```diff
diff --git a/include/rodio_hip.h b/include/rodio_hip.h
--- a/include/rodio_hip.h
+++ b/include/rodio_hip.h
@@ -278,6 +278,9 @@
     uint32_t general_kernel;
     uint32_t ragged_pair;
     uint32_t mix_first;
+    uint32_t takeovers_granted;
+    uint32_t takeovers_denied;
+    uint32_t takeovers_completed;
 } rh_rlm_geometry_info;
 rh_status rh_rlm_geometry(rh_rlm *p, rh_rlm_geometry_info *info);
 
diff --git a/rodio_amd/_lib.py b/rodio_amd/_lib.py
--- a/rodio_amd/_lib.py
+++ b/rodio_amd/_lib.py
@@ -52,7 +52,8 @@
 
 class RlmGeometry(C.Structure):
     _fields_ = [(n, C.c_uint32) for n in ("threads", "frames_per_lane", "ring_stages", "stage_kib", "lds_bytes",
-                                           "lookback_tiles", "resident_waves_per_cu", "n_tiles", "general_kernel", "ragged_pair", "mix_first")]
+                                           "lookback_tiles", "resident_waves_per_cu", "n_tiles", "general_kernel", "ragged_pair", "mix_first",
+                                           "takeovers_granted", "takeovers_denied", "takeovers_completed")]
 
 
 vp, sz, u32, u64, i32, f32 = C.c_void_p, C.c_size_t, C.c_uint32, C.c_uint64, C.c_int32, C.c_float
diff --git a/rodio_amd/csrc/rh_common.h b/rodio_amd/csrc/rh_common.h
--- a/rodio_amd/csrc/rh_common.h
+++ b/rodio_amd/csrc/rh_common.h
@@ -17,7 +17,7 @@
 
 enum Knob {
     K_AGC_SEQ, K_AGC_VEC, K_BIQUAD_NO_FALLBACK, K_BIQUAD_SEQ, K_BIQUAD_R, K_BIQUAD_NW, K_BIQUAD_WGS, K_LIMIT_SEQ, K_LIMIT_R, K_LIMIT_NW, K_LIMIT_WGS, K_LIMIT_GRID,
-    K_LIMIT_SKEW, K_LIMIT_NIO, K_LIMIT_INIT, K_SCAN_DMA_TOP, K_SCAN_SPIN_LIMIT, K_NO_HYBRID, K_NO_TICKET_SHARDS, K_PROF_DUMP, K_HOST_ALLOC, K_NO_MIX_FIRST, K_MIX_U, K_NO_CHUNK, K_CHUNK_HALF, K_AUTOTUNE_LOG, K_RAG_RESIDENT, K_RAG_TWO_KERNELS, K_AGC_SEGMENTS, K_RS_PIPE, K_DASP_I64_VIA_F64, K_MIX_GROUPS, K_CLASSES_SIDE_BY_SIDE, K_AGC_FUSED_R4, K_STREAM_UPLOAD_ALWAYS, K_STREAM_NO_REJOIN, K_NO_SBLK, K_SBLK_KV, K_SBLK_NO_OVERLAP, K_CLASSES_ONE_BY_ONE, K_CLASSES_ONE_WAVE, K_WIDE_GENERAL, K_PCM_NO_TILE, K_PCM_TILE_KB, K_LERP_IEEE_DIV, K_COUNTER_JUMP, K_STREAM_START, K_COUNT
+    K_LIMIT_SKEW, K_LIMIT_NIO, K_LIMIT_INIT, K_SCAN_DMA_TOP, K_SCAN_SPIN_LIMIT, K_NO_HYBRID, K_NO_TICKET_SHARDS, K_PROF_DUMP, K_HOST_ALLOC, K_NO_MIX_FIRST, K_MIX_U, K_NO_CHUNK, K_CHUNK_HALF, K_AUTOTUNE_LOG, K_RAG_RESIDENT, K_RAG_TWO_KERNELS, K_AGC_SEGMENTS, K_RS_PIPE, K_DASP_I64_VIA_F64, K_MIX_GROUPS, K_CLASSES_SIDE_BY_SIDE, K_AGC_FUSED_R4, K_STREAM_UPLOAD_ALWAYS, K_STREAM_NO_REJOIN, K_NO_SBLK, K_SBLK_KV, K_SBLK_NO_OVERLAP, K_CLASSES_ONE_BY_ONE, K_CLASSES_ONE_WAVE, K_WIDE_GENERAL, K_PCM_NO_TILE, K_PCM_TILE_KB, K_LERP_IEEE_DIV, K_COUNTER_JUMP, K_STREAM_START, K_CHUNK_NO_TAKEOVER, K_CHUNK_TAKE_MIN, K_CHUNK_LAG, K_COUNT
 };
 const char *knob(Knob k);
 void load_knobs();
diff --git a/rodio_amd/csrc/rh_pipeline.hip b/rodio_amd/csrc/rh_pipeline.hip
--- a/rodio_amd/csrc/rh_pipeline.hip
+++ b/rodio_amd/csrc/rh_pipeline.hip
@@ -1300,19 +1300,178 @@
 #define RH_CPH(i)
 #define RH_CPH_DECL
 #endif
-template <int R, int C, int KV>
-__device__ __forceinline__ void rlm_chunk_tile(const Params &p, const ChunkArgs &q, const uint32_t block) {
+#if defined(RH_CHUNK_DIAG) && RH_CHUNK_DIAG == 4
+__device__ unsigned long long g_chunk_ends[4096 * 8];
+#define RH_CEND(i) { if (lane == 0 && tile < 4096) __hip_atomic_store(g_chunk_ends + (uint64_t)tile * 8 + (i), (unsigned long long)wall_clock64(), __ATOMIC_RELAXED, __HIP_MEMORY_SCOPE_AGENT); }
+#define RH_CEND_WHERE { if (lane == 0 && tile < 4096) g_chunk_ends[(uint64_t)tile * 8 + 4] = ((unsigned long long)__builtin_amdgcn_s_getreg(20 | (3 << 11)) << 32) | __builtin_amdgcn_s_getreg(4 | (15 << 11)); }
+#else
+#define RH_CEND(i)
+#define RH_CEND_WHERE
+#endif
+struct ChunkTake {
+    unsigned long long *box;
+    unsigned long long *slot;
+    uint32_t *map;
+    uint32_t *count;
+    uint32_t on;
+    uint32_t take_min;
+    uint32_t lag;
+};
+constexpr uint32_t kTakeMin = 8;
+constexpr uint32_t kTakeReq = 1u, kTakeClosed = 2u, kTakeGrant = 0x80000000u;
+typedef __attribute__((address_space(4))) const uint64_t chunk_cu64;
+typedef __attribute__((address_space(4))) const float chunk_cf32;
+template <int KV, int K0, int KN>
+__device__ __forceinline__ void chunk_stage_rows(const void *data, const uint32_t (&goff)[KV], bool lin, uint32_t lds_stage) {
+    if (lin) {
+        glds16_run<KN>(data, goff[K0], lds_stage + K0 * 1024);
+    } else {
+#pragma unroll
+        for (int k = 0; k < KN; ++k) glds16(data, goff[K0 + k], lds_stage + (K0 + k) * 1024);
+    }
+}
+template <int KV, int K0, int KN, typename Early>
+__device__ __forceinline__ void chunk_sum_rows(chunk_cu64 *desc, chunk_cf32 *dgain, const lds_u8 *lds, uint32_t lds0, int lane, const uint32_t (&goff)[KV], bool lin,
+                                               uint32_t s0, uint32_t S, uint32_t st, bool primed, bool lag, v4f (&acc)[KV], Early &&early) {
+    constexpr uint32_t kStage = KV * 1024;
+    s0 = (uint32_t)__builtin_amdgcn_readfirstlane((int)s0);
+    S = (uint32_t)__builtin_amdgcn_readfirstlane((int)S);
+    st = (uint32_t)__builtin_amdgcn_readfirstlane((int)st);
+    if (!primed) {
+        if (s0 < S) chunk_stage_rows<KV, K0, KN>((const void *)(uintptr_t)desc[4 * (uint64_t)s0], goff, lin, lds0 + st * kStage);
+        if (s0 + 1 < S) chunk_stage_rows<KV, K0, KN>((const void *)(uintptr_t)desc[4 * (uint64_t)(s0 + 1)], goff, lin, lds0 + (st ^ 1u) * kStage);
+    }
+    float g_next = s0 < S ? dgain[8 * (uint64_t)s0 + 4] : 0.f;
+    uint32_t s_ = s0;
+    for (; s_ + 1 < S; ++s_) {
+        const float g = g_next;
+        g_next = dgain[8 * (uint64_t)(s_ + 1) + 4];
+        wait_vm<KN>();
+        const lds_u8 *buf = lds + st * kStage;
+        v4f v[KN];
+#pragma unroll
+        for (int k = 0; k < KN; ++k) v[k] = *(const lds_f4 *)(buf + (K0 + k) * 1024 + lane * 16);
+        asm volatile("s_waitcnt lgkmcnt(0)" ::: "memory");
+        if (s_ + 2 < S) chunk_stage_rows<KV, K0, KN>((const void *)(uintptr_t)desc[4 * (uint64_t)(s_ + 2)], goff, lin, lds0 + st * kStage);
+#pragma unroll
+        for (int k = 0; k < KN; ++k) {
+            acc[K0 + k].x = fma_(g, v[k].x, acc[K0 + k].x);
+            acc[K0 + k].y = fma_(g, v[k].y, acc[K0 + k].y);
+            acc[K0 + k].z = fma_(g, v[k].z, acc[K0 + k].z);
+            acc[K0 + k].w = fma_(g, v[k].w, acc[K0 + k].w);
+        }
+        if (lag) __builtin_amdgcn_s_sleep(64);
+        st ^= 1u;
+    }
+    if (s_ < S) {
+        early();
+        wait_vm<0>();
+        const lds_u8 *buf = lds + st * kStage;
+        v4f v[KN];
+#pragma unroll
+        for (int k = 0; k < KN; ++k) v[k] = *(const lds_f4 *)(buf + (K0 + k) * 1024 + lane * 16);
+        asm volatile("s_waitcnt lgkmcnt(0)" ::: "memory");
+#pragma unroll
+        for (int k = 0; k < KN; ++k) {
+            acc[K0 + k].x = fma_(g_next, v[k].x, acc[K0 + k].x);
+            acc[K0 + k].y = fma_(g_next, v[k].y, acc[K0 + k].y);
+            acc[K0 + k].z = fma_(g_next, v[k].z, acc[K0 + k].z);
+            acc[K0 + k].w = fma_(g_next, v[k].w, acc[K0 + k].w);
+        }
+    }
+}
+template <int KV>
+__device__ __forceinline__ void chunk_thief(const Params &p, const ChunkTake &t, const uint32_t tile, const uint32_t nvec, lds_u8 *lds, uint32_t lds0, int lane) {
+    constexpr int KN = KV / 2;
+    chunk_cu64 *const desc = (chunk_cu64 *)(uintptr_t)p.srcs;
+    chunk_cf32 *const dgain = (chunk_cf32 *)(uintptr_t)p.srcs;
+    const uint32_t epoch = p.epoch, S = p.n_sources;
+    const unsigned long long req = ((unsigned long long)epoch << 32) | kTakeReq;
+    wait_vm<0>();
+    const uint32_t nw = (p.n_tiles + 31u) / 32u;
+    const uint32_t h = tile * 0x9E3779B1u;
+    for (int round = 0; round < 2; ++round) {
+        const uint32_t wi = ((h >> 16) + (uint32_t)round * 7u + (uint32_t)lane) % nw;
+        uint32_t w = (uint32_t)lane < nw ? __hip_atomic_load(t.map + wi, __ATOMIC_RELAXED, __HIP_MEMORY_SCOPE_AGENT) : 0u;
+        const uint32_t rot = (h >> 8) & 31u;
+        w = (w >> rot) | (w << ((32u - rot) & 31u));
+        const unsigned long long any = __ballot(w != 0u);
+        if (!any) return;
+        const int src_lane = __builtin_ctzll(any);
+        const uint32_t wv = (uint32_t)__builtin_amdgcn_readlane((int)w, src_lane), wiv = (uint32_t)__builtin_amdgcn_readlane((int)wi, src_lane);
+        const uint32_t victim = wiv * 32u + (((uint32_t)__builtin_ctz(wv) + rot) & 31u);
+        if (victim >= p.n_tiles || victim == tile) continue;
+        unsigned long long *box = t.box + (uint64_t)victim * 2;
+        uint32_t won = 0;
+        if (lane == 0) {
+            const unsigned long long old = __hip_atomic_load(box, __ATOMIC_RELAXED, __HIP_MEMORY_SCOPE_AGENT);
+            if ((uint32_t)(old >> 32) != epoch) won = atomicCAS(box, old, req) == old ? 1u : 0u;
+        }
+        if (!__builtin_amdgcn_readfirstlane((int)won)) continue;
+        unsigned long long a = req;
+        for (uint32_t spins = 0; a == req; ++spins) {
+            if (spins > kSpinLimit) return;
+            __builtin_amdgcn_s_sleep(8);
+            a = __hip_atomic_load(box, __ATOMIC_RELAXED, __HIP_MEMORY_SCOPE_AGENT);
+        }
+        const uint32_t state = (uint32_t)__builtin_amdgcn_readfirstlane((int)(uint32_t)a);
+        if (!(state & kTakeGrant)) {
+            if (lane == 0) atomicAdd(t.count + 1, 1u);
+            continue;
+        }
+        const uint32_t k0 = state & ~kTakeGrant;
+        unsigned long long *const give = t.slot + (uint64_t)victim * (2 * kTakeSlots) + (uint32_t)lane, *const back = give + kTakeSlots;
+        v4f acc[KV];
+        {
+            unsigned long long gv[KN * 4];
+            bool ok = false;
+            for (uint32_t spins = 0; !__all(ok); ++spins) {
+                if (spins > kSpinLimit) return;
+                if (spins) __builtin_amdgcn_s_sleep(2);
+                ok = true;
+#pragma unroll
+                for (int j = 0; j < KN * 4; ++j) {
+                    gv[j] = __hip_atomic_load(give + j * 64, __ATOMIC_RELAXED, __HIP_MEMORY_SCOPE_AGENT);
+                    ok = ok && (uint32_t)(gv[j] >> 32) == epoch;
+                }
+            }
+#pragma unroll
+            for (int k = 0; k < KN; ++k) acc[KN + k] = v4f{__uint_as_float((uint32_t)gv[4 * k]), __uint_as_float((uint32_t)gv[4 * k + 1]), __uint_as_float((uint32_t)gv[4 * k + 2]), __uint_as_float((uint32_t)gv[4 * k + 3])};
+        }
+        uint32_t goff[KV];
+        const uint32_t v0 = victim * (KV * 64);
+#pragma unroll
+        for (int k = 0; k < KV; ++k) {
+            uint32_t j = v0 + (uint32_t)k * 64 + lane;
+            j = j < nvec ? j : nvec - 1;
+            goff[k] = j * 16;
+        }
+        const bool lin = v0 + (uint32_t)(KV * 64) <= nvec;
+        asm volatile("s_waitcnt lgkmcnt(0)" ::: "memory");
+        chunk_sum_rows<KV, KN, KN>(desc, dgain, lds, lds0, lane, goff, lin, k0, S, 0u, false, false, acc, [] {});
+#pragma unroll
+        for (int k = 0; k < KN; ++k) {
+            const float e[4] = {acc[KN + k].x, acc[KN + k].y, acc[KN + k].z, acc[KN + k].w};
+#pragma unroll
+            for (int w4 = 0; w4 < 4; ++w4) __hip_atomic_store(back + (4 * k + w4) * 64, ((unsigned long long)epoch << 32) | __float_as_uint(e[w4]), __ATOMIC_RELAXED, __HIP_MEMORY_SCOPE_AGENT);
+        }
+        wait_vm<0>();
+    }
+}
+template <int R, int C, int KV, bool TAKE>
+__device__ __forceinline__ void rlm_chunk_tile(const Params &p, const ChunkArgs &q, const ChunkTake &tk, const uint32_t block) {
     typedef Chan<C> CH;
     typedef typename CH::V V;
     constexpr int NS = 2, H = 4;
     constexpr uint32_t FB = CH::kFB;
     constexpr uint32_t kStage = KV * 1024, P = kStage / FB;
+    static_assert(!TAKE || (KV % 2 == 0 && (KV / 2) * 4 * 64 <= (int)kTakeSlots && kStage >= 1024), "take-over: half the sub-rows fit a slot; the mailbox poll lands in the image");
     constexpr uint32_t MB = NS * kStage + 64;
     __shared__ __attribute__((aligned(1024))) unsigned char smem[MB + kStage + 64];
     lds_u8 *const lds = (lds_u8 *)smem;
     const uint32_t lds0 = (uint32_t)(uintptr_t)lds;
-    typedef __attribute__((address_space(4))) const uint64_t cu64;
-    typedef __attribute__((address_space(4))) const float cf32;
+    typedef chunk_cu64 cu64;
+    typedef chunk_cf32 cf32;
     typedef __attribute__((address_space(4))) const uint32_t cu32;
     cu64 *const desc = (cu64 *)(uintptr_t)p.srcs;
     cf32 *const dgain = (cf32 *)(uintptr_t)p.srcs;
@@ -1324,6 +1483,14 @@
         tile = x + 8u * k;
         if (tile >= p.n_tiles) return;
     }
+    RH_CEND(0)
+    RH_CEND_WHERE
+#if defined(RH_CHUNK_RAGSIM) || (defined(RH_CHUNK_DIAG) && RH_CHUNK_DIAG < 3)
+    const bool take_on = false;
+#else
+    const bool take_on = TAKE && tk.on != 0;
+#endif
+    if (TAKE && take_on && lane == 0) atomicOr(tk.map + (tile >> 5), 1u << (tile & 31u));
 #ifdef RH_CHUNK_RAGSIM
     const uint32_t Ns = p.eq_frames;
     const uint32_t S = 2u * tile < p.n_tiles ? p.n_sources : (uint32_t)(((uint64_t)p.n_sources * 2u * (p.n_tiles - tile)) / p.n_tiles);
@@ -1426,20 +1593,61 @@
     v4f acc[KV];
 #pragma unroll
     for (int k = 0; k < KV; ++k) acc[k] = v4f{0.f, 0.f, 0.f, 0.f};
+    unsigned long long hv_early = 0, gv_early[2 * C];
+#pragma unroll
+    for (int k = 0; k < 2 * C; ++k) gv_early[k] = 0;
+    bool granted = false;
+    auto early = [&]() {
+        if constexpr (TAKE) {
+            if (tile > 0 && lane < H * C) hv_early = __hip_atomic_load((RH_GLB const unsigned long long *)(uintptr_t)a_halo_poll, __ATOMIC_RELAXED, __HIP_MEMORY_SCOPE_AGENT);
+            if (tile > 0 && want_look) {
+#pragma unroll
+                for (int k = 0; k < 2 * C; ++k) gv_early[k] = __hip_atomic_load((RH_GLB const unsigned long long *)(uintptr_t)a_gran_poll + k, __ATOMIC_RELAXED, __HIP_MEMORY_SCOPE_AGENT);
+            }
+            if (take_on && lane == 0) {
+                atomicAnd(tk.map + (tile >> 5), ~(1u << (tile & 31u)));
+                if (!granted) __hip_atomic_store(tk.box + (uint64_t)tile * 2, ((unsigned long long)p.epoch << 32) | kTakeClosed, __ATOMIC_RELAXED, __HIP_MEMORY_SCOPE_AGENT);
+            }
+        }
+    };
     {
         uint32_t st = 0;
         float g_next = S ? dgain[4] : 0.f;
-        for (uint32_t s_ = 0; s_ < S; ++s_) {
+        const bool lag = TAKE && take_on && tk.lag && tile % tk.lag == 0;
+        bool polled = false, box_open = take_on, grant = false;
+        uint32_t s_ = 0;
+        for (; s_ + 1 < S; ++s_) {
             const float g = g_next;
-            g_next = s_ + 1 < S ? dgain[8 * (uint64_t)(s_ + 1) + 4] : 0.f;
-            if (s_ + 1 < S) wait_vm<KV>();
-            else wait_vm<0>();
+            g_next = dgain[8 * (uint64_t)(s_ + 1) + 4];
+            wait_vm<KV>();
             const lds_u8 *buf = lds + st * kStage;
             v4f v[KV];
 #pragma unroll
             for (int k = 0; k < KV; ++k) v[k] = *(const lds_f4 *)(buf + k * 1024 + lane * 16);
+            if constexpr (TAKE) {
+                if (polled) {
+                    const unsigned long long w = *(const RH_LDS unsigned long long *)(lds + MB);
+                    const uint32_t w_tag = (uint32_t)__builtin_amdgcn_readfirstlane((int)(uint32_t)(w >> 32)), w_state = (uint32_t)__builtin_amdgcn_readfirstlane((int)(uint32_t)w);
+                    polled = false;
+                    if (w_tag == p.epoch && w_state == kTakeReq) {
+                        box_open = false;
+                        grant = S - (s_ + 1) >= tk.take_min;
+                        if (!grant && lane == 0)
+                            __hip_atomic_store((RH_GLB unsigned long long *)tk.box + (uint64_t)tile * 2, ((unsigned long long)p.epoch << 32) | kTakeClosed, __ATOMIC_RELAXED, __HIP_MEMORY_SCOPE_AGENT);
+                    }
+                }
+            }
             asm volatile("s_waitcnt lgkmcnt(0)" ::: "memory");
-            if (s_ + 2 < S) stage_source(s_ + 2, st);
+            if constexpr (TAKE) {
+                if (box_open && (s_ & 3u) == 0 && s_ + 1 + tk.take_min < S) {
+                    glds16_sc1((const void *)(tk.box + (uint64_t)tile * 2), 0u, lds0 + MB);
+                    polled = true;
+                }
+            }
+            if (s_ + 2 < S) {
+                if (TAKE && grant) chunk_stage_rows<KV, 0, KV / 2>((const void *)(uintptr_t)desc[4 * (uint64_t)(s_ + 2)], goff, lin, lds0 + st * kStage);
+                else stage_source(s_ + 2, st);
+            }
 #pragma unroll
             for (int k = 0; k < KV; ++k) {
                 acc[k].x = fma_(g, v[k].x, acc[k].x);
@@ -1447,7 +1655,79 @@
                 acc[k].z = fma_(g, v[k].z, acc[k].z);
                 acc[k].w = fma_(g, v[k].w, acc[k].w);
             }
+            if constexpr (TAKE) {
+                if (lag) __builtin_amdgcn_s_sleep(64);
+            }
             st ^= 1u;
+            if (TAKE && grant) break;
+        }
+        if (s_ < S && !(TAKE && grant)) {
+            early();
+            wait_vm<0>();
+            const lds_u8 *buf = lds + st * kStage;
+            v4f v[KV];
+#pragma unroll
+            for (int k = 0; k < KV; ++k) v[k] = *(const lds_f4 *)(buf + k * 1024 + lane * 16);
+            asm volatile("s_waitcnt lgkmcnt(0)" ::: "memory");
+#pragma unroll
+            for (int k = 0; k < KV; ++k) {
+                acc[k].x = fma_(g_next, v[k].x, acc[k].x);
+                acc[k].y = fma_(g_next, v[k].y, acc[k].y);
+                acc[k].z = fma_(g_next, v[k].z, acc[k].z);
+                acc[k].w = fma_(g_next, v[k].w, acc[k].w);
+            }
+        }
+        if constexpr (TAKE) {
+            if (grant) {
+                constexpr int KN = KV / 2;
+                granted = true;
+                unsigned long long *const give = tk.slot + (uint64_t)tile * (2 * kTakeSlots) + (uint32_t)lane;
+#pragma unroll
+                for (int k = 0; k < KN; ++k) {
+                    const float e[4] = {acc[KN + k].x, acc[KN + k].y, acc[KN + k].z, acc[KN + k].w};
+#pragma unroll
+                    for (int w4 = 0; w4 < 4; ++w4) __hip_atomic_store(give + (4 * k + w4) * 64, ((unsigned long long)p.epoch << 32) | __float_as_uint(e[w4]), __ATOMIC_RELAXED, __HIP_MEMORY_SCOPE_AGENT);
+                }
+                if (lane == 0) {
+                    __hip_atomic_store(tk.box + (uint64_t)tile * 2, ((unsigned long long)p.epoch << 32) | kTakeGrant | (s_ + 1), __ATOMIC_RELAXED, __HIP_MEMORY_SCOPE_AGENT);
+                    atomicAdd(tk.count, 1u);
+                }
+                chunk_sum_rows<KV, 0, KN>(desc, dgain, lds, lds0, lane, goff, lin, s_ + 1, S, st, true, lag, acc, early);
+            }
+        }
+    }
+    RH_CEND(1)
+    bool dead = false;
+    if constexpr (TAKE) {
+        if (granted) {
+            constexpr int KN = KV / 2;
+            const unsigned long long *const back = tk.slot + (uint64_t)tile * (2 * kTakeSlots) + kTakeSlots + (uint32_t)lane;
+            unsigned long long gv[KN * 4];
+            bool ok = false;
+            for (uint32_t spins = 0; !__all(ok); ++spins) {
+                if (spins > kSpinLimit) {
+                    if (lane == 0) atomicOr(p.status, 1u);
+                    dead = true;
+                    break;
+                }
+                if (spins) __builtin_amdgcn_s_sleep(2);
+                ok = true;
+#pragma unroll
+                for (int j = 0; j < KN * 4; ++j) {
+                    gv[j] = __hip_atomic_load(back + j * 64, __ATOMIC_RELAXED, __HIP_MEMORY_SCOPE_AGENT);
+                    ok = ok && (uint32_t)(gv[j] >> 32) == p.epoch;
+                }
+            }
+#pragma unroll
+            for (int k = 0; k < KN; ++k) {
+                const float nanv = __builtin_nanf("");
+                acc[KN + k] = dead ? v4f{nanv, nanv, nanv, nanv}
+                                   : v4f{__uint_as_float((uint32_t)gv[4 * k]), __uint_as_float((uint32_t)gv[4 * k + 1]), __uint_as_float((uint32_t)gv[4 * k + 2]), __uint_as_float((uint32_t)gv[4 * k + 3])};
+            }
+            if (lane == 0) {
+                __hip_atomic_store(tk.box + (uint64_t)tile * 2, ((unsigned long long)p.epoch << 32) | kTakeClosed, __ATOMIC_RELAXED, __HIP_MEMORY_SCOPE_AGENT);
+                if (!dead) atomicAdd(tk.count + 2, 1u);
+            }
         }
     }
     RH_CPH_DECL
@@ -1471,14 +1751,13 @@
 #pragma unroll
     for (int k = 0; k < KV; ++k) *(lds_f4 *)(lds + MB + (uint32_t)(k * 64 + lane) * 16) = acc[k];
     if (lane == 0) *(lds_f4 *)(lds + MB + kStage) = v4f{0.f, 0.f, 0.f, 0.f};
-    bool dead = false;
     if (tile == 0) {
         if (lane < H * C) *(RH_LDS float *)(lds + MB - H * FB + lane * 4) = 0.0f;
     } else {
         const bool want = lane < H * C;
         const unsigned long long *hp = (const unsigned long long *)(uintptr_t)a_halo_poll;
-        unsigned long long hv = 0;
-        bool ok = false;
+        unsigned long long hv = hv_early;
+        bool ok = TAKE && (uint32_t)(hv >> 32) == epoch_v;
         uint32_t spins = 0;
         while (true) {
             if (want && !ok) {
@@ -1610,9 +1889,12 @@
         const bool want = want_look != 0;
         const unsigned long long *gp = (const unsigned long long *)(uintptr_t)a_gran_poll;
         unsigned long long gv[2 * C];
-#pragma unroll
-        for (int k = 0; k < 2 * C; ++k) gv[k] = 0;
-        bool ok = false;
+        bool ok = TAKE;
+#pragma unroll
+        for (int k = 0; k < 2 * C; ++k) {
+            gv[k] = gv_early[k];
+            ok = ok && ((uint32_t)(gv[k] >> 32) == epoch_v);
+        }
         uint32_t spins = 0;
         while (true) {
             if (want && !ok) {
@@ -1684,10 +1966,18 @@
         }
     }
     RH_CPH(4)
+    RH_CEND(2)
+    if constexpr (TAKE) {
+        if (take_on) {
+            asm volatile("s_waitcnt lgkmcnt(0)" ::: "memory");
+            chunk_thief<KV>(p, tk, tile, nvec, lds, lds0, lane);
+        }
+    }
+    RH_CEND(3)
 }
 template <int R, int C, int KV>
-__global__ __launch_bounds__(64, 2) void k_rlm_chunk(const Params p, const ChunkArgs q) {
-    rlm_chunk_tile<R, C, KV>(p, q, blockIdx.x);
+__global__ __launch_bounds__(64, 2) void k_rlm_chunk(const Params p, const ChunkArgs q, const ChunkTake tk) {
+    rlm_chunk_tile<R, C, KV, true>(p, q, tk, blockIdx.x);
 }
 template <int R, int C, int KV>
 __global__ __launch_bounds__(64, 2) void k_rlm_chunk_multi(const ChunkMulti m) {
@@ -1712,7 +2002,7 @@
 #pragma unroll
         for (uint32_t i = 0; i < sizeof(ChunkArgs) / 4; ++i) dq[i] = wq[i];
     }
-    rlm_chunk_tile<R, C, KV>(p, q, blockIdx.x - b0);
+    rlm_chunk_tile<R, C, KV, false>(p, q, ChunkTake{}, blockIdx.x - b0);
 }
 
 #if defined(RH_CLS_DIAG) && RH_CLS_DIAG == 9
@@ -2614,6 +2904,11 @@
     return RH_OK;
 }
 
+#if defined(RH_CHUNK_DIAG) && RH_CHUNK_DIAG == 4
+extern "C" int rh_debug_chunk_ends(unsigned long long *dst, size_t n) {
+    return (int)hipMemcpyFromSymbol(dst, HIP_SYMBOL(g_chunk_ends), n * sizeof(unsigned long long), 0, hipMemcpyDeviceToHost);
+}
+#endif
 #if defined(RH_CLS_DIAG) && RH_CLS_DIAG == 9
 extern "C" int rh_debug_cls_stamps(unsigned long long *dst, size_t n) {
     return (int)hipMemcpyFromSymbol(dst, HIP_SYMBOL(g_cls_stamp), n * sizeof(unsigned long long), 0, hipMemcpyDeviceToHost);
@@ -2753,7 +3048,15 @@
             return RH_OK;
         }
         const uint32_t cgrid = k.direct ? c.n_tiles : (c.n_tiles + 7u) & ~7u;
-        void *cargs[] = {&k, &ca};
+        ChunkTake tk{};
+        tk.box = c.d_box;
+        tk.slot = c.d_slot;
+        tk.map = c.d_map;
+        tk.count = p->d_ctl + 4;
+        tk.on = (c.take && !rh::knob(rh::K_CHUNK_NO_TAKEOVER)) ? 1u : 0u;
+        tk.take_min = rh::knob(rh::K_CHUNK_TAKE_MIN) ? (uint32_t)std::max(1l, atol(rh::knob(rh::K_CHUNK_TAKE_MIN))) : kTakeMin;
+        tk.lag = rh::knob(rh::K_CHUNK_LAG) ? (uint32_t)std::max(0, atoi(rh::knob(rh::K_CHUNK_LAG))) : 0u;
+        void *cargs[] = {&k, &ca, &tk};
         const hipError_t ce = hipLaunchKernel(c.fn, dim3(cgrid), dim3(64), cargs, 0, s);
         if (ce != hipSuccess) {
             rh::set_hip_error(ce, "k_rlm_chunk launch");
diff --git a/rodio_amd/csrc/rh_pipeline_internal.h b/rodio_amd/csrc/rh_pipeline_internal.h
--- a/rodio_amd/csrc/rh_pipeline_internal.h
+++ b/rodio_amd/csrc/rh_pipeline_internal.h
@@ -29,6 +29,7 @@
 #endif
 constexpr int kMaxR = 20;
 constexpr int kGroupLag = RH_CARRY_DEFER;
+constexpr size_t kTakeSlots = 1024;
 constexpr int kMaxLook = 32;
 constexpr uint32_t kSpinLimit = 1u << 22;
 
@@ -170,6 +171,11 @@
     float *d_look = nullptr;
     unsigned long long *d_halo = nullptr;
     unsigned long long *d_gran = nullptr;
+    unsigned long long *d_box = nullptr;
+    unsigned long long *d_slot = nullptr;
+    uint32_t *d_map = nullptr;
+    size_t cap_take = 0;
+    bool take = false;
     size_t cap_tiles = 0, cap_look = 0;
     uint32_t n_tiles = 0, J = 0, frames = 0;
     int resident_per_cu = 0;
diff --git a/rodio_amd/csrc/rh_pipeline_plan.hip b/rodio_amd/csrc/rh_pipeline_plan.hip
--- a/rodio_amd/csrc/rh_pipeline_plan.hip
+++ b/rodio_amd/csrc/rh_pipeline_plan.hip
@@ -59,6 +59,8 @@
     RH_HIP_TRY(launch_retag(p->d_gran, p->gran_words, r, s));
     RH_HIP_TRY(launch_retag(p->chunk.d_halo, p->chunk.cap_tiles * 8, r, s));
     RH_HIP_TRY(launch_retag(p->chunk.d_gran, p->chunk.cap_tiles * 4, r, s));
+    RH_HIP_TRY(launch_retag(p->chunk.d_box, p->chunk.cap_take * 2, r, s));
+    RH_HIP_TRY(launch_retag(p->chunk.d_slot, p->chunk.cap_take * 2 * kTakeSlots, r, s));
     sblk_retag(p, s, r);
     RH_CHECK_LAUNCH();
     return RH_OK;
@@ -332,6 +334,21 @@
         RH_HIP_TRY(rh::fill_now(c.d_gran, 0, (size_t)tiles * 32));
         c.cap_tiles = (size_t)tiles;
     }
+    c.take = tiles <= 4ull * (uint64_t)rh::g_num_cus * (uint64_t)c.resident_per_cu;
+    if (c.take && (size_t)tiles > c.cap_take) {
+        if (c.d_box) RH_HIP_TRY(hipFree(c.d_box));
+        if (c.d_slot) RH_HIP_TRY(hipFree(c.d_slot));
+        if (c.d_map) RH_HIP_TRY(hipFree(c.d_map));
+        c.d_box = nullptr, c.d_slot = nullptr, c.d_map = nullptr, c.cap_take = 0;
+        const size_t map_bytes = (((size_t)tiles + 31) / 32) * 4;
+        RH_HIP_TRY(hipMalloc(reinterpret_cast<void **>(&c.d_box), (size_t)tiles * 16));
+        RH_HIP_TRY(hipMalloc(reinterpret_cast<void **>(&c.d_slot), (size_t)tiles * 2 * kTakeSlots * 8));
+        RH_HIP_TRY(hipMalloc(reinterpret_cast<void **>(&c.d_map), map_bytes));
+        RH_HIP_TRY(rh::fill_now(c.d_box, 0, (size_t)tiles * 16));
+        RH_HIP_TRY(rh::fill_now(c.d_slot, 0, (size_t)tiles * 2 * kTakeSlots * 8));
+        RH_HIP_TRY(rh::fill_now(c.d_map, 0, map_bytes));
+        c.cap_take = (size_t)tiles;
+    }
     const size_t look_floats = (size_t)tiles * J * 4;
     if (look_floats > c.cap_look) {
         if (c.d_look) RH_HIP_TRY(hipFree(c.d_look));
@@ -608,6 +625,9 @@
     if (p->chunk.d_look) (void)hipFree(p->chunk.d_look);
     if (p->chunk.d_halo) (void)hipFree(p->chunk.d_halo);
     if (p->chunk.d_gran) (void)hipFree(p->chunk.d_gran);
+    if (p->chunk.d_box) (void)hipFree(p->chunk.d_box);
+    if (p->chunk.d_slot) (void)hipFree(p->chunk.d_slot);
+    if (p->chunk.d_map) (void)hipFree(p->chunk.d_map);
     if (p->d_prof) (void)hipFree(p->d_prof);
     if (p->d_replay) (void)hipFree(p->d_replay);
     for (int k = 0; k < 2; ++k)
@@ -1038,7 +1058,16 @@
     info->general_kernel = (pl.general || p->plan == &p->pair) ? 1u : 0u;
     info->ragged_pair = p->plan == &p->pair ? 1u : 0u;
     info->mix_first = (p->pre_filter && p->plan == &p->fast) ? 1u : mix_first_applies(p, pl, p->n_sources, false, false) ? (p->chunk.ok ? 2u : 1u) : 0u;
-    return RH_OK;
-}
-
-}
+    uint32_t take[3] = {0, 0, 0};
+    if (p->chunk.cap_take) {
+        const rh_status w = wait_idle(p);
+        if (w != RH_OK) return w;
+        RH_HIP_TRY(hipMemcpy(take, p->d_ctl + 4, sizeof(take), hipMemcpyDeviceToHost));
+    }
+    info->takeovers_granted = take[0];
+    info->takeovers_denied = take[1];
+    info->takeovers_completed = take[2];
+    return RH_OK;
+}
+
+}
diff --git a/rodio_amd/csrc/rh_runtime.hip b/rodio_amd/csrc/rh_runtime.hip
--- a/rodio_amd/csrc/rh_runtime.hip
+++ b/rodio_amd/csrc/rh_runtime.hip
@@ -21,7 +21,7 @@
 namespace {
 const char *const kKnobNames[K_COUNT] = {"RH_AGC_SEQ", "RH_AGC_VEC", "RH_BIQUAD_NO_FALLBACK", "RH_BIQUAD_SEQ", "RH_BIQUAD_R", "RH_BIQUAD_NW", "RH_BIQUAD_WGS", "RH_LIMIT_SEQ",
                                          "RH_LIMIT_R", "RH_LIMIT_NW", "RH_LIMIT_WGS", "RH_LIMIT_GRID", "RH_LIMIT_SKEW", "RH_LIMIT_NIO", "RH_LIMIT_INIT", "RH_SCAN_DMA_TOP", "RH_SCAN_SPIN_LIMIT", "RH_NO_HYBRID",
-                                         "RH_NO_TICKET_SHARDS", "RH_PROF_DUMP", "RH_HOST_ALLOC", "RH_NO_MIX_FIRST", "RH_MIX_U", "RH_NO_CHUNK", "RH_CHUNK_HALF", "RH_AUTOTUNE_LOG", "RH_RAG_RESIDENT", "RH_RAG_TWO_KERNELS", "RH_AGC_SEGMENTS", "RH_RS_PIPE", "RH_DASP_I64_VIA_F64", "RH_MIX_GROUPS", "RH_CLASSES_SIDE_BY_SIDE", "RH_AGC_FUSED_R4", "RH_STREAM_UPLOAD_ALWAYS", "RH_STREAM_NO_REJOIN", "RH_NO_SBLK", "RH_SBLK_KV", "RH_SBLK_NO_OVERLAP", "RH_CLASSES_ONE_BY_ONE", "RH_CLASSES_ONE_WAVE", "RH_WIDE_GENERAL", "RH_PCM_NO_TILE", "RH_PCM_TILE_KB", "RH_LERP_IEEE_DIV", "RH_COUNTER_JUMP", "RH_STREAM_START"};
+                                         "RH_NO_TICKET_SHARDS", "RH_PROF_DUMP", "RH_HOST_ALLOC", "RH_NO_MIX_FIRST", "RH_MIX_U", "RH_NO_CHUNK", "RH_CHUNK_HALF", "RH_AUTOTUNE_LOG", "RH_RAG_RESIDENT", "RH_RAG_TWO_KERNELS", "RH_AGC_SEGMENTS", "RH_RS_PIPE", "RH_DASP_I64_VIA_F64", "RH_MIX_GROUPS", "RH_CLASSES_SIDE_BY_SIDE", "RH_AGC_FUSED_R4", "RH_STREAM_UPLOAD_ALWAYS", "RH_STREAM_NO_REJOIN", "RH_NO_SBLK", "RH_SBLK_KV", "RH_SBLK_NO_OVERLAP", "RH_CLASSES_ONE_BY_ONE", "RH_CLASSES_ONE_WAVE", "RH_WIDE_GENERAL", "RH_PCM_NO_TILE", "RH_PCM_TILE_KB", "RH_LERP_IEEE_DIV", "RH_COUNTER_JUMP", "RH_STREAM_START", "RH_CHUNK_NO_TAKEOVER", "RH_CHUNK_TAKE_MIN", "RH_CHUNK_LAG"};
 std::string g_knob_val[K_COUNT];
 bool g_knob_set[K_COUNT];
 CounterJump g_jump{false, 0, 0, 0};
diff --git a/rust/rodio-hip/src/ffi.rs b/rust/rodio-hip/src/ffi.rs
--- a/rust/rodio-hip/src/ffi.rs
+++ b/rust/rodio-hip/src/ffi.rs
@@ -103,6 +103,9 @@
     pub general_kernel: u32,
     pub ragged_pair: u32,
     pub mix_first: u32,
+    pub takeovers_granted: u32,
+    pub takeovers_denied: u32,
+    pub takeovers_completed: u32,
 }
 
 extern "C" {
```

Result: slower. 1.638 million Msamples/s (-2.5%).
